# yccyenchicheng/p2pvg

Hardware: NVIDIA H100
Metric: frames/sec (train step, device-timed) MovingMNIST 64x64 seq30 (higher is better)
Workload: dtype bf16

## Files before the change

p2pvg_b200/csrc/conv_gemm.cu:

```cuda

#include "tc_common.cuh"

namespace {

using namespace tc;

struct Geom {
  int N, H, W;
  int Ck, Cn;
  int M;
  int Ntot;
  int bh128, bn128;
  int bh64, bn64;
  int bw64;
  int imgs_per_group;
  int add_bf16;
  int bres;
  int swap;
  int ks, st, sgn;
};

__device__ __forceinline__ void pix_block(int pb, int P, int H, int W, int bh, int bn, int& n0, int& y0) {
  const int HW = H * W;
  if (HW >= P) {
    const int bpi = HW / P;
    n0 = pb / bpi;
    y0 = (pb - n0 * bpi) * bh;
  } else {
    n0 = pb * bn;
    y0 = 0;
  }
}

__device__ __forceinline__ void addend_load64(float4 (&a4)[16], const float* base, long long elem_off, bool is_bf16) {
  if (is_bf16) {
    const uint4* p = reinterpret_cast<const uint4*>(reinterpret_cast<const bf16*>(base) + elem_off);
#pragma unroll
    for (int j = 0; j < 8; j++) {
      const uint4 r = p[j];
      a4[j] = make_float4(__uint_as_float(r.x), __uint_as_float(r.y), __uint_as_float(r.z), __uint_as_float(r.w));
    }
  } else {
    const float4* p = reinterpret_cast<const float4*>(base + elem_off);
#pragma unroll
    for (int j = 0; j < 16; j++) a4[j] = p[j];
  }
}
__device__ __forceinline__ void addend_add32(float (&f)[32], const float4 (&a4)[16], int h, bool is_bf16) {
  if (is_bf16) {
#pragma unroll
    for (int j = 0; j < 4; j++) {
      const float4 r = a4[4 * h + j];
      float v[8];
      unpack16<bf16>(make_uint4(__float_as_uint(r.x), __float_as_uint(r.y), __float_as_uint(r.z), __float_as_uint(r.w)), v);
#pragma unroll
      for (int i = 0; i < 8; i++) f[8 * j + i] += v[i];
    }
  } else {
#pragma unroll
    for (int j = 0; j < 8; j++) {
      const float4 x4 = a4[8 * h + j];
      f[4 * j] += x4.x; f[4 * j + 1] += x4.y; f[4 * j + 2] += x4.z; f[4 * j + 3] += x4.w;
    }
  }
}

template <int KIND, int BN, bool STAT, bool EVAL = false>
__global__ void __launch_bounds__(NUM_THREADS, 1)
conv_gemm_kernel(const __grid_constant__ CUtensorMap tmA, const __grid_constant__ CUtensorMap tmB, void* __restrict__ Cv, int c_bf16,
                 long long ldc, Geom g, int accumulate, const float* __restrict__ bias, const float* __restrict__ addend,
                 const int* __restrict__ grp_src, float* __restrict__ partial, int kb_per_split, int splits,
                 float2* __restrict__ stat_partial, const float* __restrict__ eval_scale, const float* __restrict__ eval_shift, int act) {
  using C_ = Cfg<BN>;
  constexpr bool A_MN = (KIND == 1), B_MN = (KIND != 0);
  extern __shared__ uint8_t smem_raw[];
  const Smem sm = smem_setup<BN>(smem_raw);
  const bool bres = (KIND == 0) && (BN == 64) && g.bres != 0;

  const int warp = threadIdx.x >> 5, lane = threadIdx.x & 31;
  const int tiles_m = (g.M + BLOCK_M - 1) / BLOCK_M, tiles_n = (g.Ntot + BN - 1) / BN;
  const int tiles_mn = tiles_m * tiles_n;
  const int phases = (KIND == 2) ? 4 : 1;
  const int num_tiles = tiles_mn * splits * phases;
  const int cchunks = g.Ck / 64;
  const int nkb_total = (KIND == 0) ? g.ks * g.ks * cchunks : (KIND == 2) ? 4 * cchunks : (g.N * g.H * g.W + 63) / 64;

  if (warp >= 8) {
    regs_producer();
    if (warp == 8 && lane == 0) {
      uint32_t it = 0;
      if (bres) {
        mbar_expect_tx(sm.bres_bar, (uint32_t)(g.ks * g.ks) * 64 * 128);
        for (int tap = 0; tap < g.ks * g.ks; tap++) tma_load_2d(&tmB, sm.bres_bar, sm.ring + tap * 64 * 128, tap * 64, 0);
      }
      for (int t = blockIdx.x; t < num_tiles; t += gridDim.x) {
        const int ph = (KIND == 2) ? (t & 3) : 0;
        const int t2 = (KIND == 2) ? (t >> 2) : t;
        const int z = (splits == 1) ? 0 : t2 / tiles_mn, r = t2 - z * tiles_mn;
        const int mt = (tiles_n == 1) ? r : r / tiles_n, nt = (tiles_n == 1) ? 0 : r - mt * tiles_n;
        const int n0 = nt * BN;
        const int kb0 = z * kb_per_split, kb1 = min(kb0 + kb_per_split, nkb_total);
        int pn0 = 0, py0 = 0;
        if (KIND != 1) pix_block(mt, 128, g.H, g.W, g.bh128, g.bn128, pn0, py0);
        const int pa = ph >> 1, pb_ = ph & 1;
        int kn0 = 0, ky0 = 0, kx0 = 0;
        int t_kh = 0, t_kw = 0, t_cc = 0;
        int qc0[BN / 64], qdx[BN / 64], qdy[BN / 64];
        int mc0[2] = {0, 0}, mdx[2] = {0, 0}, mdy[2] = {0, 0};
        if (KIND == 1) {
          if (g.bw64 < g.W) {
            const int per_row = g.W / g.bw64;
            const int rowi = kb0 / per_row;
            kx0 = (kb0 - rowi * per_row) * g.bw64;
            kn0 = rowi / g.H;
            ky0 = rowi - kn0 * g.H;
          } else {
            pix_block(kb0, 64, g.H, g.W, g.bh64, g.bn64, kn0, ky0);
          }
#pragma unroll
          for (int q = 0; q < BN / 64; q++) {
            const int nb = n0 + 64 * q;
            const int tap = nb / g.Cn;
            const int kh = tap / g.ks;
            qc0[q] = nb - tap * g.Cn;
            qdx[q] = tap - kh * g.ks - 1;
            qdy[q] = kh - 1;
          }
          if (g.swap) {
#pragma unroll
            for (int q = 0; q < 2; q++) {
              const int mb = mt * BLOCK_M + 64 * q;
              int tap = mb / g.Cn;
              if (tap >= g.ks * g.ks) tap = g.ks * g.ks - 1;
              const int kh = tap / g.ks;
              mc0[q] = mb < g.M ? mb - tap * g.Cn : 0;
              mdx[q] = tap - kh * g.ks - 1;
              mdy[q] = kh - 1;
            }
          }
        }
        for (int kb = kb0; kb < kb1; kb++, it++) {
          const int s = bres ? (int)(it % BRES_STAGES) : (int)(it % C_::STAGES);
          const uint32_t par = (bres ? (it / BRES_STAGES) : (it / C_::STAGES)) & 1;
          mbar_wait(&sm.empty_bar[s], par ^ 1);
          uint8_t* sa = bres ? sm.ring + BRES_B_BYTES + s * A_STAGE_BYTES : sm.ring + s * C_::STAGE_BYTES;
          uint8_t* sb = sa + A_STAGE_BYTES;
          mbar_expect_tx(&sm.full_bar[s], bres ? A_STAGE_BYTES : C_::STAGE_BYTES);
          if (KIND == 0) {
            tma_load_4d(&tmA, &sm.full_bar[s], sa, t_cc * 64, g.sgn * (t_kw - 1), g.st * py0 + g.sgn * (t_kh - 1), pn0);
            if (!bres) tma_load_2d(&tmB, &sm.full_bar[s], sb, kb * 64, n0);
            if (++t_cc == cchunks) { t_cc = 0; if (++t_kw == g.ks) { t_kw = 0; t_kh++; } }
          } else if (KIND == 2) {
            const int tq = t_kh, c0 = t_cc * 64;
            if (++t_cc == cchunks) { t_cc = 0; t_kh++; }
            const int i = tq >> 1, j = tq & 1;
            const int dy = i == 0 ? 0 : (pa ? 1 : -1), ky = i == 0 ? pa + 1 : (pa ? 0 : 3);
            const int dx = j == 0 ? 0 : (pb_ ? 1 : -1), kx = j == 0 ? pb_ + 1 : (pb_ ? 0 : 3);
            tma_load_4d(&tmA, &sm.full_bar[s], sa, c0, dx, py0 + dy, pn0);
#pragma unroll
            for (int q = 0; q < BN / 64; q++)
              tma_load_2d(&tmB, &sm.full_bar[s], sb + q * 64 * 128, (ky * 4 + kx) * g.Cn + n0 + 64 * q, c0);
          } else {
            const int m0 = mt * BLOCK_M;
            if (g.swap) {
              tma_load_4d(&tmA, &sm.full_bar[s], sa, mc0[0], g.st * kx0 + mdx[0], g.st * ky0 + mdy[0], kn0);
              tma_load_4d(&tmA, &sm.full_bar[s], sa + 64 * 128, mc0[1], g.st * kx0 + mdx[1], g.st * ky0 + mdy[1], kn0);
#pragma unroll
              for (int q = 0; q < BN / 64; q++) tma_load_2d(&tmB, &sm.full_bar[s], sb + q * 64 * 128, n0 + 64 * q, kb * 64);
            } else {
              tma_load_2d(&tmA, &sm.full_bar[s], sa, m0, kb * 64);
              tma_load_2d(&tmA, &sm.full_bar[s], sa + 64 * 128, m0 + 64, kb * 64);
#pragma unroll
              for (int q = 0; q < BN / 64; q++)
                tma_load_4d(&tmB, &sm.full_bar[s], sb + q * 64 * 128, qc0[q], g.st * kx0 + qdx[q], g.st * ky0 + qdy[q], kn0);
            }
            if (g.bw64 < g.W) {
              kx0 += g.bw64;
              if (kx0 >= g.W) { kx0 = 0; if (++ky0 >= g.H) { ky0 = 0; kn0++; } }
            } else if (g.H * g.W >= 64) {
              ky0 += g.bh64;
              if (ky0 >= g.H) { ky0 = 0; kn0++; }
            } else {
              kn0 += g.bn64;
            }
          }
        }
      }
    }
  } else if (warp >= 4) {
    regs_worker();
    mma_loop<false, BN, A_MN, B_MN>(sm, num_tiles, tiles_mn, splits, kb_per_split, nkb_total, bres);
  } else {
    regs_worker();
    const int q = warp;
    __shared__ float bias_s[2 * BN];
    __shared__ float2 stat_s[STAT ? 2 * 4 * BN : 1];
    constexpr bool do_stat = STAT;
    __shared__ float ev_s[EVAL ? 2 * 2 * BN : 1];
    const bool row_major_store = !STAT && !EVAL && KIND != 1 && c_bf16 && !accumulate && addend == nullptr;
    uint32_t lt = 0;
    for (int t = blockIdx.x; t < num_tiles; t += gridDim.x, lt++) {
      const int ph = (KIND == 2) ? (t & 3) : 0;
      const int t2 = (KIND == 2) ? (t >> 2) : t;
      const int z = (splits == 1) ? 0 : t2 / tiles_mn, r = t2 - z * tiles_mn;
      const int mt = (tiles_n == 1) ? r : r / tiles_n, nt = (tiles_n == 1) ? 0 : r - mt * tiles_n;
      const int n0 = nt * BN;
      const uint32_t acc = lt & 1;
      const int rt = q * 32 + lane;
      long long out_row = (long long)mt * BLOCK_M + rt;
      long long add_row = 0;
      bool row_ok = out_row < g.M;
      if (KIND == 2) {
        int pn0, py0;
        pix_block(mt, 128, g.H, g.W, g.bh128, g.bn128, pn0, py0);
        const int HW = g.H * g.W;
        int nn, yy, xx;
        if (HW >= 128) { nn = 0; yy = rt / g.W; xx = rt - yy * g.W; }
        else { nn = rt / HW; const int rem = rt - nn * HW; yy = rem / g.W; xx = rem - yy * g.W; }
        const int n = pn0 + nn, y = py0 + yy;
        row_ok = (n < g.N) && (y < g.H);
        const int oy = 2 * y + (ph >> 1), ox = 2 * xx + (ph & 1);
        out_row = ((long long)n * (2 * g.H) + oy) * (2 * g.W) + ox;
        if (addend && row_ok) {
          const int n2 = grp_src[n / g.imgs_per_group] * g.imgs_per_group + (n % g.imgs_per_group);
          add_row = ((long long)n2 * (2 * g.H) + oy) * (2 * g.W) + ox;
        }
      }
      if (KIND == 0 && addend && row_ok) {
        const int HW = g.H * g.W;
        const int n = (int)(out_row / HW);
        const int n2 = grp_src[n / g.imgs_per_group] * g.imgs_per_group + (n % g.imgs_per_group);
        add_row = (long long)n2 * HW + (out_row - (long long)n * HW);
      }
      if (EVAL) {
        stage_cols<BN>(ev_s + acc * 2 * BN, eval_scale, n0, g.Ntot);
        stage_cols<BN>(ev_s + acc * 2 * BN + BN, eval_shift, n0, g.Ntot);
        if (bias == nullptr) epi_bar_sync();
      }
      if (bias != nullptr) {
        stage_cols<BN>(bias_s + acc * BN, bias, n0, g.Ntot);
        epi_bar_sync();
      }
      const bool use_add = (KIND != 1) && addend != nullptr && row_ok;
      const long long aoff0 = add_row * g.Ntot + n0;
      const bool abf = g.add_bf16 != 0;
      if (row_major_store) {
        constexpr int LPR = BN / 8, RPI = 32 / LPR;
        const int sub = lane / LPR, cl = (lane % LPR) * 8;
        const bool col_ok = n0 + cl < g.Ntot;
        bf16* cbase = reinterpret_cast<bf16*>(Cv) + n0 + cl;
        mbar_wait(sm.acc_full_bar, lt & 1);
#pragma unroll
        for (int i = 0; i < 32 / RPI; i++) {
          const int src = i * RPI + sub;
          const long long orow = __shfl_sync(0xffffffffu, out_row, src);
          const bool ok = __shfl_sync(0xffffffffu, (int)row_ok, src) != 0;
          const float* s = sm.accs + (q * 32 + src) * C_::ACC_LD + cl;
          const float4 x0 = *reinterpret_cast<const float4*>(s), x1 = *reinterpret_cast<const float4*>(s + 4);
          if (i == 32 / RPI - 1) {
            __syncwarp();
            if (lane == 0) mbar_arrive(sm.acc_empty_bar);
          }
          if (!ok || !col_ok) continue;
          float f[8] = {x0.x, x0.y, x0.z, x0.w, x1.x, x1.y, x1.z, x1.w};
          if (bias) {
#pragma unroll
            for (int j = 0; j < 8; j++) f[j] += bias_s[acc * BN + cl + j];
          }
          *reinterpret_cast<uint4*>(cbase + orow * ldc) = pack16<bf16>(f);
        }
        continue;
      }
      float4 a4[16];
      if (use_add) addend_load64(a4, addend, aoff0, abf);
      mbar_wait(sm.acc_full_bar, lt & 1);
#pragma unroll 1
      for (int pr = 0; pr < BN / 64; pr++) {
        if (pr > 0 && use_add) addend_load64(a4, addend, aoff0 + pr * 64, abf);
#pragma unroll
        for (int h = 0; h < 2; h++) {
          const int c = pr * 2 + h;
          float f[32];
          read_chunk<BN>(sm, rt, c, f);
          const int nbase = n0 + c * 32;
          if (nbase >= g.Ntot) continue;
          if (!row_ok && !do_stat) continue;
          if (KIND == 1 && partial != nullptr) {
            float* dst = partial + ((long long)z * g.M + out_row) * g.Ntot + nbase;
#pragma unroll
            for (int j = 0; j < 32; j += 8)
              st_global_256(dst + j, __float_as_uint(f[j]), __float_as_uint(f[j + 1]), __float_as_uint(f[j + 2]), __float_as_uint(f[j + 3]),
                            __float_as_uint(f[j + 4]), __float_as_uint(f[j + 5]), __float_as_uint(f[j + 6]), __float_as_uint(f[j + 7]));
            continue;
          }
          if (bias) add_staged32(f, bias_s + acc * BN + c * 32);
          if (use_add) addend_add32(f, a4, h, abf);
          if (EVAL) {
            const float* sc = ev_s + acc * 2 * BN + c * 32;
#pragma unroll
            for (int j = 0; j < 32; j++) {
              float y = fmaf(f[j], sc[j], sc[BN + j]);
              if (act == P2PVG_ACT_LRELU) y = y > 0.f ? y : 0.2f * y;
              else if (act == P2PVG_ACT_TANH) y = tanhf(y);
              f[j] = y;
            }
          }
          if (STAT) {
            float s1[32], s2[32];
#pragma unroll
            for (int j = 0; j < 32; j++) {
              const float r = row_ok ? (c_bf16 ? bf16_round(f[j]) : f[j]) : 0.f;
              s1[j] = r;
              s2[j] = r * r;
            }
            const float cs = warp_colsum32(s1, lane), cq = warp_colsum32(s2, lane);
            stat_s[(acc * 4 + q) * BN + c * 32 + lane] = make_float2(cs, cq);
            if (!row_ok) continue;
          }
          if (c_bf16) store_row32<bf16, false>(reinterpret_cast<bf16*>(Cv) + out_row * ldc + nbase, f, accumulate, 32);
          else store_row32<float, false>(reinterpret_cast<float*>(Cv) + out_row * ldc + nbase, f, accumulate, 32);
        }
      }
      if (STAT) {
        epi_bar_sync();
        float2* dst = stat_partial + ((long long)mt * phases + ph) * g.Ntot + n0;
        for (int i = q * 32 + lane; i < BN; i += 128) {
          if (n0 + i >= g.Ntot) continue;
          const float2 a = stat_s[(acc * 4 + 0) * BN + i], b = stat_s[(acc * 4 + 1) * BN + i];
          const float2 c2 = stat_s[(acc * 4 + 2) * BN + i], d = stat_s[(acc * 4 + 3) * BN + i];
          dst[i] = make_float2((a.x + b.x) + (c2.x + d.x), (a.y + b.y) + (c2.y + d.y));
        }
      }
    }
  }
}

int map4d(CUtensorMap* m, const void* base, int N, int Hm, int Wm, int C, int bw, int bh, int bn, int s) {
  cuuint64_t dims[4] = {(cuuint64_t)C, (cuuint64_t)Wm, (cuuint64_t)Hm, (cuuint64_t)N};
  cuuint64_t strides[3] = {(cuuint64_t)C * 2, (cuuint64_t)Wm * C * 2, (cuuint64_t)Hm * Wm * C * 2};
  cuuint32_t box[4] = {64, (cuuint32_t)(bw * s), (cuuint32_t)(bh * s), (cuuint32_t)bn};
  cuuint32_t es[4] = {1, (cuuint32_t)s, (cuuint32_t)s, 1};
  CUresult r = driver().encode(m, CU_TENSOR_MAP_DATA_TYPE_BFLOAT16, 4, const_cast<void*>(base), dims, strides, box, es, CU_TENSOR_MAP_INTERLEAVE_NONE,
                     CU_TENSOR_MAP_SWIZZLE_128B, CU_TENSOR_MAP_L2_PROMOTION_L2_256B, CU_TENSOR_MAP_FLOAT_OOB_FILL_NONE);
  if (r != CUDA_SUCCESS) {
    p2pvg_set_error("conv_gemm: 4-D tensor map failed (%d): N=%d H=%d W=%d C=%d box=(%d,%d,%d) s=%d", (int)r, N, Hm, Wm, C, bw, bh, bn, s);
    return P2PVG_ERR_CUDA;
  }
  return P2PVG_OK;
}

bool box_for(int P, int H, int W, int& bh, int& bn) {
  const int HW = H * W;
  if (HW >= P) {
    if (P % W != 0 || (H % (P / W)) != 0) return false;
    bh = P / W;
    bn = 1;
  } else {
    if (P % HW != 0) return false;
    bh = H;
    bn = P / HW;
  }
  return bh * 2 <= 256 && W * 2 <= 256 && bn <= 256;
}

struct EvalEpi {
  const float* scale = nullptr;
  const float* shift = nullptr;
  int act = 0;
};

template <int KIND, int BN, bool STAT, bool EVAL>
int launch_t(const CUtensorMap& ta, const CUtensorMap& tb, void* C, int c_dtype, long long ldc, const Geom& g, int accumulate,
             const float* bias, const float* addend, const int* grp_src, float* partial, int splits, int kb_per_split, cudaStream_t st,
             float2* stat_partial, const EvalEpi& ev) {
  const long long tiles = (long long)cdiv(g.M, BLOCK_M) * cdiv(g.Ntot, BN) * splits * (KIND == 2 ? 4 : 1);
  return launch_persistent<conv_gemm_kernel<KIND, BN, STAT, EVAL>, BN>(tiles, st, "conv_gemm", ta, tb, C, (int)(c_dtype == P2PVG_BF16), ldc, g,
                                                                       accumulate, bias, addend, grp_src, partial, kb_per_split, splits,
                                                                       stat_partial, ev.scale, ev.shift, ev.act);
}

template <int KIND, int BN>
int launch(const CUtensorMap& ta, const CUtensorMap& tb, void* C, int c_dtype, long long ldc, const Geom& g, int accumulate,
           const float* bias, const float* addend, const int* grp_src, float* partial, int splits, int kb_per_split, cudaStream_t st,
           float2* stat_partial = nullptr, const EvalEpi& ev = EvalEpi()) {
  if (KIND != 1 && ev.scale != nullptr) return launch_t<KIND, BN, false, (KIND != 1)>(ta, tb, C, c_dtype, ldc, g, accumulate, bias, addend, grp_src, partial, splits, kb_per_split, st, nullptr, ev);
  if (KIND != 1 && stat_partial != nullptr) return launch_t<KIND, BN, (KIND != 1), false>(ta, tb, C, c_dtype, ldc, g, accumulate, bias, addend, grp_src, partial, splits, kb_per_split, st, stat_partial, ev);
  return launch_t<KIND, BN, false, false>(ta, tb, C, c_dtype, ldc, g, accumulate, bias, addend, grp_src, partial, splits, kb_per_split, st, nullptr, ev);
}

}

int p2pvg_conv_gemm_impl(int kind, const void* a, const void* b, long long ldb, void* c, int c_dtype, long long ldc, int N, int H, int W,
                         int Ck, int Cn, int Cm, const float* bias, const float* addend, const int* grp_src, int imgs_per_group,
                         int accumulate, void* ws, size_t ws_bytes, void* stat_partial_v, int addend_dtype, const float* eval_scale,
                         const float* eval_shift, int act, cudaStream_t st) {
  float2* stat_partial = reinterpret_cast<float2*>(stat_partial_v);
  EvalEpi ev;
  ev.scale = eval_scale; ev.shift = eval_shift; ev.act = act;
  P2PVG_REQUIRE(driver().encode != nullptr, P2PVG_ERR_UNSUPPORTED, "conv_gemm: cuTensorMapEncodeTiled unavailable");
  P2PVG_REQUIRE(kind >= 0 && kind <= 5, P2PVG_ERR_BAD_ARG, "conv_gemm: bad kind %d", kind);
  if (eval_scale != nullptr) {
    P2PVG_REQUIRE(kind == 0 || kind == 2, P2PVG_ERR_BAD_ARG, "conv_gemm: the eval-BatchNorm epilogue belongs to kinds 0 and 2");
    P2PVG_REQUIRE(eval_shift != nullptr, P2PVG_ERR_BAD_ARG, "conv_gemm: eval_scale without eval_shift");
    P2PVG_REQUIRE(stat_partial == nullptr, P2PVG_ERR_BAD_ARG, "conv_gemm: the eval-BatchNorm epilogue excludes fwd_stat_partial");
    P2PVG_REQUIRE(!accumulate, P2PVG_ERR_BAD_ARG, "conv_gemm: the eval-BatchNorm epilogue does not accumulate");
    P2PVG_REQUIRE(act == P2PVG_ACT_LRELU || act == P2PVG_ACT_TANH, P2PVG_ERR_BAD_ARG, "conv_gemm: eval epilogue act %d", act);
  }
  if (N <= 0) return P2PVG_OK;
  Geom g;
  g.N = N; g.H = H; g.W = W; g.Ck = Ck; g.Cn = Cn; g.imgs_per_group = imgs_per_group > 0 ? imgs_per_group : 1;
  g.add_bf16 = (addend != nullptr && addend_dtype == P2PVG_BF16) ? 1 : 0;
  g.swap = 0;
  g.bres = 0;
  g.ks = kind >= 3 ? 3 : 4; g.st = kind >= 3 ? 1 : 2; g.sgn = kind == 5 ? -1 : 1;
  const int taps = g.ks * g.ks;
  if (kind == 3 || kind == 5) kind = 0;
  if (kind == 4) kind = 1;
  g.bh128 = g.bn128 = g.bh64 = g.bn64 = 1;
  g.bw64 = W;
  bool ok;
  if (kind == 1) {
    if (W > 64 && W % 64 == 0 && W * g.st <= 256) { g.bw64 = 64; ok = true; }
    else ok = box_for(64, H, W, g.bh64, g.bn64);
  } else {
    ok = box_for(128, H, W, g.bh128, g.bn128);
  }
  ok = ok && (((uintptr_t)a | (uintptr_t)b | (uintptr_t)c) & 15) == 0;
  if (kind == 1) ok = ok && (Cn % 64 == 0) && (Cm % 8 == 0);
  else ok = ok && (Ck % 64 == 0) && (Cn % 32 == 0) && (ldb % 8 == 0);
  if (kind == 2 || addend != nullptr) ok = ok && (Cn % 64 == 0);
  if (!ok) {
    p2pvg_set_error("conv_gemm: shape not supported by the pixel-box tiling (kind=%d N=%d H=%d W=%d Ck=%d Cn=%d)", kind, N, H, W, Ck, Cn);
    return P2PVG_ERR_UNSUPPORTED;
  }
  CUtensorMap ta, tb;
  int rc;
  const long long pix = (long long)N * H * W;
  if (kind == 0) {
    g.M = (int)pix; g.Ntot = Cn;
    rc = map4d(&ta, a, N, g.st * H, g.st * W, Ck, W, g.bh128, g.bn128, g.st);
    if (rc) return rc;
    const int BN = Cn > 64 ? 128 : 64;
    rc = map2d(&tb, b, (long long)taps * Ck, Cn, ldb, BN);
    if (rc) return rc;
    const int nkb = taps * (Ck / 64);
    g.bres = (BN == 64 && Cn == 64 && Ck == 64 && taps <= 9) ? 1 : 0;
    if (BN == 128) return launch<0, 128>(ta, tb, c, c_dtype, ldc, g, accumulate, bias, addend, grp_src, nullptr, 1, nkb, st, stat_partial, ev);
    return launch<0, 64>(ta, tb, c, c_dtype, ldc, g, accumulate, bias, addend, grp_src, nullptr, 1, nkb, st, stat_partial, ev);
  }
  if (kind == 2) {
    g.M = (int)pix; g.Ntot = Cn;
    rc = map4d(&ta, a, N, H, W, Ck, W, g.bh128, g.bn128, 1);
    if (rc) return rc;
    rc = map2d(&tb, b, 16LL * Cn, Ck, ldb, 64);
    if (rc) return rc;
    const int nkb = 4 * (Ck / 64);
    const int BN = Cn > 64 ? 128 : 64;
    if (BN == 128) return launch<2, 128>(ta, tb, c, c_dtype, ldc, g, accumulate, bias, addend, grp_src, nullptr, 1, nkb, st, stat_partial, ev);
    return launch<2, 64>(ta, tb, c, c_dtype, ldc, g, accumulate, bias, addend, grp_src, nullptr, 1, nkb, st, stat_partial, ev);
  }
  P2PVG_REQUIRE(c_dtype == P2PVG_F32, P2PVG_ERR_BAD_ARG, "conv_gemm kind 1 writes fp32");
  P2PVG_REQUIRE(stat_partial == nullptr, P2PVG_ERR_BAD_ARG, "conv_gemm: BatchNorm statistics belong to the forward / data-gradient kinds");
  g.Ck = 64;
  const int nkb = (int)((pix + 63) / 64);
  g.swap = (Cm == 64 && nkb >= 16 && ws != nullptr && (size_t)2 * taps * Cn * Cm * sizeof(float) <= ws_bytes) ? 1 : 0;
  if (g.swap) {
    g.M = taps * Cn; g.Ntot = Cm;
    rc = map4d(&ta, b, N, g.st * H, g.st * W, Cn, g.bw64, g.bh64, g.bn64, g.st);
    if (rc) return rc;
    rc = map2d(&tb, a, Cm, pix, Cm, 64);
    if (rc) return rc;
  } else {
    g.M = Cm; g.Ntot = taps * Cn;
    rc = map2d(&ta, a, Cm, pix, Cm, 64);
    if (rc) return rc;
    rc = map4d(&tb, b, N, g.st * H, g.st * W, Cn, g.bw64, g.bh64, g.bn64, g.st);
    if (rc) return rc;
  }
  const int BN = (g.Ntot % 128 == 0) ? 128 : 64;
  const long long tiles = (long long)cdiv(g.M, BLOCK_M) * cdiv(g.Ntot, BN);
  int splits = g.swap ? 2 : 1;
  {
    double best = 1e300;
    const int maxs = nkb / 8 < 64 ? nkb / 8 : 64;
    const int smin = g.swap ? 2 : 1;
    for (int s = smin; s <= (maxs < smin ? smin : maxs); s++) {
      const int kb = cdiv(nkb, s), se = cdiv(nkb, kb);
      if (se > 1 && (ws == nullptr || (size_t)se * g.M * g.Ntot * sizeof(float) > ws_bytes)) continue;
      const long long rounds = cdiv((long long)tiles * se, driver().sms);
      double cost = (double)rounds * (kb + 8.0);
      if (se > 1) cost += (double)se * g.M * g.Ntot * 8.0 / 6.0e12 / (0.22e-6 * BN / 128);
      if (cost < best) { best = cost; splits = se; }
    }
  }
  int kbps = cdiv(nkb, splits);
  splits = cdiv(nkb, kbps);
  float* partial = splits > 1 ? reinterpret_cast<float*>(ws) : nullptr;
  if (BN == 128) rc = launch<1, 128>(ta, tb, c, c_dtype, ldc, g, accumulate, nullptr, nullptr, nullptr, partial, splits, kbps, st);
  else rc = launch<1, 64>(ta, tb, c, c_dtype, ldc, g, accumulate, nullptr, nullptr, nullptr, partial, splits, kbps, st);
  if (rc) return rc;
  if (splits > 1)
    return p2pvg_splitk_reduce(partial, splits, c, P2PVG_F32, ldc, Cm, taps * Cn, accumulate, nullptr, nullptr, 0, g.swap, st);
  P2PVG_REQUIRE(!g.swap, P2PVG_ERR_UNSUPPORTED, "conv_gemm kind 1 (swapped roles) needs the split-K workspace");
  return P2PVG_OK;
}
```

p2pvg_b200/csrc/tc_common.cuh:

```cuda
#pragma once
#include <cuda.h>

#include "common.cuh"

namespace tc {

__device__ __forceinline__ uint32_t smem_u32(const void* p) { return (uint32_t)__cvta_generic_to_shared(p); }

__device__ __forceinline__ void mbar_init(uint64_t* bar, uint32_t count) {
  asm volatile("mbarrier.init.shared::cta.b64 [%0], %1;" ::"r"(smem_u32(bar)), "r"(count));
}
__device__ __forceinline__ void mbar_expect_tx(uint64_t* bar, uint32_t bytes) {
  asm volatile("mbarrier.arrive.expect_tx.shared::cta.b64 _, [%0], %1;" ::"r"(smem_u32(bar)), "r"(bytes) : "memory");
}
__device__ __forceinline__ void mbar_wait(uint64_t* bar, uint32_t parity) {
  asm volatile(
      "{\n\t"
      ".reg .pred P1;\n\t"
      "WAIT_LOOP:\n\t"
      "mbarrier.try_wait.parity.shared::cta.b64 P1, [%0], %1;\n\t"
      "@P1 bra DONE;\n\t"
      "bra WAIT_LOOP;\n\t"
      "DONE:\n\t"
      "}" ::"r"(smem_u32(bar)),
      "r"(parity)
      : "memory");
}
__device__ __forceinline__ void tma_load_2d(const CUtensorMap* desc, uint64_t* bar, void* smem_dst, int c0, int c1) {
  asm volatile(
      "cp.async.bulk.tensor.2d.shared::cluster.global.mbarrier::complete_tx::bytes [%0], [%1, {%3, %4}], [%2];" ::"r"(
          smem_u32(smem_dst)),
      "l"(reinterpret_cast<uint64_t>(desc)), "r"(smem_u32(bar)), "r"(c0), "r"(c1)
      : "memory");
}
__device__ __forceinline__ void wgmma_fence() { asm volatile("wgmma.fence.sync.aligned;" ::: "memory"); }
__device__ __forceinline__ void wgmma_commit() { asm volatile("wgmma.commit_group.sync.aligned;" ::: "memory"); }
template <int N>
__device__ __forceinline__ void wgmma_wait() { asm volatile("wgmma.wait_group.sync.aligned %0;" ::"n"(N) : "memory"); }
template <int N>
__device__ __forceinline__ void fence_regs(float (&r)[N]) {
#pragma unroll
  for (int i = 0; i < N; i++) asm volatile("" : "+f"(r[i])::"memory");
}
template <int TA, int TB>
__device__ __forceinline__ void wgmma_bf16_n64(float* d, uint64_t desc_a, uint64_t desc_b, uint32_t scale_d) {
  asm volatile(
      "{\n\t.reg .pred p;\n\tsetp.ne.b32 p, %34, 0;\n\t"
      "wgmma.mma_async.sync.aligned.m64n64k16.f32.bf16.bf16 "
      "{%0, %1, %2, %3, %4, %5, %6, %7, %8, %9, %10, %11, %12, %13, %14, %15, %16, %17, %18, %19, %20, %21, %22, %23, %24, %25, %26, %27, %28, %29, %30, %31}, %32, %33, p, 1, 1, %35, %36;\n\t}"
      : "+f"(d[0]), "+f"(d[1]), "+f"(d[2]), "+f"(d[3]), "+f"(d[4]), "+f"(d[5]), "+f"(d[6]), "+f"(d[7]), "+f"(d[8]), "+f"(d[9]), "+f"(d[10]), "+f"(d[11]), "+f"(d[12]), "+f"(d[13]), "+f"(d[14]), "+f"(d[15]), "+f"(d[16]), "+f"(d[17]), "+f"(d[18]), "+f"(d[19]), "+f"(d[20]), "+f"(d[21]), "+f"(d[22]), "+f"(d[23]), "+f"(d[24]), "+f"(d[25]), "+f"(d[26]), "+f"(d[27]), "+f"(d[28]), "+f"(d[29]), "+f"(d[30]), "+f"(d[31])
      : "l"(desc_a), "l"(desc_b), "r"(scale_d), "n"(TA), "n"(TB));
}
template <int TA, int TB>
__device__ __forceinline__ void wgmma_bf16_n128(float* d, uint64_t desc_a, uint64_t desc_b, uint32_t scale_d) {
  asm volatile(
      "{\n\t.reg .pred p;\n\tsetp.ne.b32 p, %66, 0;\n\t"
      "wgmma.mma_async.sync.aligned.m64n128k16.f32.bf16.bf16 "
      "{%0, %1, %2, %3, %4, %5, %6, %7, %8, %9, %10, %11, %12, %13, %14, %15, %16, %17, %18, %19, %20, %21, %22, %23, %24, %25, %26, %27, %28, %29, %30, %31, %32, %33, %34, %35, %36, %37, %38, %39, %40, %41, %42, %43, %44, %45, %46, %47, %48, %49, %50, %51, %52, %53, %54, %55, %56, %57, %58, %59, %60, %61, %62, %63}, %64, %65, p, 1, 1, %67, %68;\n\t}"
      : "+f"(d[0]), "+f"(d[1]), "+f"(d[2]), "+f"(d[3]), "+f"(d[4]), "+f"(d[5]), "+f"(d[6]), "+f"(d[7]), "+f"(d[8]), "+f"(d[9]), "+f"(d[10]), "+f"(d[11]), "+f"(d[12]), "+f"(d[13]), "+f"(d[14]), "+f"(d[15]), "+f"(d[16]), "+f"(d[17]), "+f"(d[18]), "+f"(d[19]), "+f"(d[20]), "+f"(d[21]), "+f"(d[22]), "+f"(d[23]), "+f"(d[24]), "+f"(d[25]), "+f"(d[26]), "+f"(d[27]), "+f"(d[28]), "+f"(d[29]), "+f"(d[30]), "+f"(d[31]), "+f"(d[32]), "+f"(d[33]), "+f"(d[34]), "+f"(d[35]), "+f"(d[36]), "+f"(d[37]), "+f"(d[38]), "+f"(d[39]), "+f"(d[40]), "+f"(d[41]), "+f"(d[42]), "+f"(d[43]), "+f"(d[44]), "+f"(d[45]), "+f"(d[46]), "+f"(d[47]), "+f"(d[48]), "+f"(d[49]), "+f"(d[50]), "+f"(d[51]), "+f"(d[52]), "+f"(d[53]), "+f"(d[54]), "+f"(d[55]), "+f"(d[56]), "+f"(d[57]), "+f"(d[58]), "+f"(d[59]), "+f"(d[60]), "+f"(d[61]), "+f"(d[62]), "+f"(d[63])
      : "l"(desc_a), "l"(desc_b), "r"(scale_d), "n"(TA), "n"(TB));
}
__device__ __forceinline__ void wgmma_tf32_n64(float* d, uint64_t desc_a, uint64_t desc_b, uint32_t scale_d) {
  asm volatile(
      "{\n\t.reg .pred p;\n\tsetp.ne.b32 p, %34, 0;\n\t"
      "wgmma.mma_async.sync.aligned.m64n64k8.f32.tf32.tf32 "
      "{%0, %1, %2, %3, %4, %5, %6, %7, %8, %9, %10, %11, %12, %13, %14, %15, %16, %17, %18, %19, %20, %21, %22, %23, %24, %25, %26, %27, %28, %29, %30, %31}, %32, %33, p, 1, 1;\n\t}"
      : "+f"(d[0]), "+f"(d[1]), "+f"(d[2]), "+f"(d[3]), "+f"(d[4]), "+f"(d[5]), "+f"(d[6]), "+f"(d[7]), "+f"(d[8]), "+f"(d[9]), "+f"(d[10]), "+f"(d[11]), "+f"(d[12]), "+f"(d[13]), "+f"(d[14]), "+f"(d[15]), "+f"(d[16]), "+f"(d[17]), "+f"(d[18]), "+f"(d[19]), "+f"(d[20]), "+f"(d[21]), "+f"(d[22]), "+f"(d[23]), "+f"(d[24]), "+f"(d[25]), "+f"(d[26]), "+f"(d[27]), "+f"(d[28]), "+f"(d[29]), "+f"(d[30]), "+f"(d[31])
      : "l"(desc_a), "l"(desc_b), "r"(scale_d));
}
__device__ __forceinline__ void wgmma_tf32_n128(float* d, uint64_t desc_a, uint64_t desc_b, uint32_t scale_d) {
  asm volatile(
      "{\n\t.reg .pred p;\n\tsetp.ne.b32 p, %66, 0;\n\t"
      "wgmma.mma_async.sync.aligned.m64n128k8.f32.tf32.tf32 "
      "{%0, %1, %2, %3, %4, %5, %6, %7, %8, %9, %10, %11, %12, %13, %14, %15, %16, %17, %18, %19, %20, %21, %22, %23, %24, %25, %26, %27, %28, %29, %30, %31, %32, %33, %34, %35, %36, %37, %38, %39, %40, %41, %42, %43, %44, %45, %46, %47, %48, %49, %50, %51, %52, %53, %54, %55, %56, %57, %58, %59, %60, %61, %62, %63}, %64, %65, p, 1, 1;\n\t}"
      : "+f"(d[0]), "+f"(d[1]), "+f"(d[2]), "+f"(d[3]), "+f"(d[4]), "+f"(d[5]), "+f"(d[6]), "+f"(d[7]), "+f"(d[8]), "+f"(d[9]), "+f"(d[10]), "+f"(d[11]), "+f"(d[12]), "+f"(d[13]), "+f"(d[14]), "+f"(d[15]), "+f"(d[16]), "+f"(d[17]), "+f"(d[18]), "+f"(d[19]), "+f"(d[20]), "+f"(d[21]), "+f"(d[22]), "+f"(d[23]), "+f"(d[24]), "+f"(d[25]), "+f"(d[26]), "+f"(d[27]), "+f"(d[28]), "+f"(d[29]), "+f"(d[30]), "+f"(d[31]), "+f"(d[32]), "+f"(d[33]), "+f"(d[34]), "+f"(d[35]), "+f"(d[36]), "+f"(d[37]), "+f"(d[38]), "+f"(d[39]), "+f"(d[40]), "+f"(d[41]), "+f"(d[42]), "+f"(d[43]), "+f"(d[44]), "+f"(d[45]), "+f"(d[46]), "+f"(d[47]), "+f"(d[48]), "+f"(d[49]), "+f"(d[50]), "+f"(d[51]), "+f"(d[52]), "+f"(d[53]), "+f"(d[54]), "+f"(d[55]), "+f"(d[56]), "+f"(d[57]), "+f"(d[58]), "+f"(d[59]), "+f"(d[60]), "+f"(d[61]), "+f"(d[62]), "+f"(d[63])
      : "l"(desc_a), "l"(desc_b), "r"(scale_d));
}
__device__ __forceinline__ void st_global_256(void* p, uint32_t a, uint32_t b, uint32_t c, uint32_t d, uint32_t e, uint32_t f, uint32_t g,
                                              uint32_t h) {
  uint4* q = reinterpret_cast<uint4*>(p);
  q[0] = make_uint4(a, b, c, d);
  q[1] = make_uint4(e, f, g, h);
}
__device__ __forceinline__ uint32_t pack_bf16x2(float lo, float hi) {
  __nv_bfloat162 v = __floats2bfloat162_rn(lo, hi);
  return *reinterpret_cast<uint32_t*>(&v);
}
__device__ __forceinline__ void regs_producer() { asm volatile("setmaxnreg.dec.sync.aligned.u32 40;"); }
__device__ __forceinline__ void regs_worker() { asm volatile("setmaxnreg.inc.sync.aligned.u32 232;"); }
__device__ __forceinline__ void epi_bar_sync() { asm volatile("bar.sync 1, 128;" ::: "memory"); }

__device__ __forceinline__ uint64_t make_desc(uint32_t smem_addr, uint32_t lbo_bytes, uint32_t sbo_bytes) {
  uint64_t d = 0;
  d |= (uint64_t)((smem_addr >> 4) & 0x3FFF);
  d |= (uint64_t)((lbo_bytes >> 4) & 0x3FFF) << 16;
  d |= (uint64_t)((sbo_bytes >> 4) & 0x3FFF) << 32;
  d |= (uint64_t)1 << 62;
  return d;
}

template <bool TF32, int BN, bool A_MN, bool B_MN>
__device__ __forceinline__ void wgmma_kblock(float (&acc)[2][BN / 2], uint64_t da, uint64_t db, bool first) {
  constexpr int UMMA_K = TF32 ? 8 : 16;
  constexpr int KSTEPS = 4;
  constexpr uint32_t A_STEP = (A_MN ? UMMA_K * 128 : 32) >> 4, B_STEP = (B_MN ? UMMA_K * 128 : 32) >> 4;
#pragma unroll
  for (int k = 0; k < KSTEPS; k++) {
    const uint32_t sc = (first && k == 0) ? 0u : 1u;
#pragma unroll
    for (int h = 0; h < 2; h++) {
      const uint64_t a = da + (uint64_t)(h * (8192 >> 4) + k * A_STEP), b = db + (uint64_t)(k * B_STEP);
      if constexpr (TF32) {
        if constexpr (BN == 128) wgmma_tf32_n128(acc[h], a, b, sc);
        else wgmma_tf32_n64(acc[h], a, b, sc);
      } else {
        if constexpr (BN == 128) wgmma_bf16_n128<A_MN ? 1 : 0, B_MN ? 1 : 0>(acc[h], a, b, sc);
        else wgmma_bf16_n64<A_MN ? 1 : 0, B_MN ? 1 : 0>(acc[h], a, b, sc);
      }
    }
  }
}

template <int BN>
__device__ __forceinline__ void acc_to_smem(const float (&acc)[2][BN / 2], float* buf, int ld, int t) {
  const int w = t >> 5, l = t & 31;
#pragma unroll
  for (int h = 0; h < 2; h++) {
    float* r0 = buf + (64 * h + 16 * w + (l >> 2)) * ld + 2 * (l & 3);
#pragma unroll
    for (int j = 0; j < BN / 8; j++) {
      *reinterpret_cast<float2*>(r0 + 8 * j) = make_float2(acc[h][4 * j], acc[h][4 * j + 1]);
      *reinterpret_cast<float2*>(r0 + 8 * ld + 8 * j) = make_float2(acc[h][4 * j + 2], acc[h][4 * j + 3]);
    }
  }
}

__device__ __forceinline__ void mbar_arrive(uint64_t* bar) {
  asm volatile("mbarrier.arrive.shared::cta.b64 _, [%0];" ::"r"(smem_u32(bar)) : "memory");
}
__device__ __forceinline__ void tma_load_4d(const CUtensorMap* desc, uint64_t* bar, void* smem_dst, int c0, int c1, int c2, int c3) {
  asm volatile(
      "cp.async.bulk.tensor.4d.shared::cluster.global.mbarrier::complete_tx::bytes [%0], [%1, {%3, %4, %5, %6}], [%2];" ::"r"(
          smem_u32(smem_dst)),
      "l"(reinterpret_cast<uint64_t>(desc)), "r"(smem_u32(bar)), "r"(c0), "r"(c1), "r"(c2), "r"(c3)
      : "memory");
}

template <int OFF>
__device__ __forceinline__ void colsum_stage(float (&v)[32], int lane) {
  const bool upper = (lane & OFF) != 0;
#pragma unroll
  for (int j = 0; j < OFF; j++) {
    const float send = upper ? v[j] : v[j + OFF];
    const float keep = upper ? v[j + OFF] : v[j];
    v[j] = keep + __shfl_xor_sync(0xffffffffu, send, OFF);
  }
  if constexpr (OFF > 1) colsum_stage<OFF / 2>(v, lane);
}
__device__ __forceinline__ float warp_colsum32(float (&v)[32], int lane) {
  colsum_stage<16>(v, lane);
  return v[0];
}
__device__ __forceinline__ float bf16_round(float x) { return __bfloat162float(__float2bfloat16_rn(x)); }

constexpr int BLOCK_M = 128;
constexpr int ROW_BYTES = 128;
constexpr int A_STAGE_BYTES = BLOCK_M * ROW_BYTES;
constexpr int NUM_THREADS = 384;

template <int BN> struct Cfg {
  static constexpr int B_STAGE_BYTES = BN * ROW_BYTES;
  static constexpr int STAGE_BYTES = A_STAGE_BYTES + B_STAGE_BYTES;
  static constexpr int STAGES = (BN == 128) ? 4 : 7;
  static constexpr int ACC_LD = BN + 4;
  static constexpr int ACC_BYTES = BLOCK_M * ACC_LD * 4;
  static constexpr int SMEM_BYTES = STAGES * STAGE_BYTES + ACC_BYTES + 1024  + 512 ;
};

constexpr int BRES_B_BYTES = 9 * 64 * 128, BRES_STAGES = 6;
static_assert(BRES_B_BYTES + BRES_STAGES * A_STAGE_BYTES <= Cfg<64>::STAGES * Cfg<64>::STAGE_BYTES, "resident weights + A ring");

struct Smem {
  uint8_t* ring;
  float* accs;
  uint64_t *full_bar, *empty_bar, *acc_full_bar, *acc_empty_bar;
  uint64_t* bres_bar;
};

template <int BN>
__device__ __forceinline__ Smem smem_setup(uint8_t* smem_raw) {
  using C_ = Cfg<BN>;
  Smem s;
  s.ring = reinterpret_cast<uint8_t*>((reinterpret_cast<uintptr_t>(smem_raw) + 1023) & ~(uintptr_t)1023);
  s.accs = reinterpret_cast<float*>(s.ring + C_::STAGES * C_::STAGE_BYTES);
  s.full_bar = reinterpret_cast<uint64_t*>(s.ring + C_::STAGES * C_::STAGE_BYTES + C_::ACC_BYTES);
  s.empty_bar = s.full_bar + C_::STAGES;
  s.acc_full_bar = s.empty_bar + C_::STAGES;
  s.acc_empty_bar = s.acc_full_bar + 1;
  s.bres_bar = s.acc_empty_bar + 1;
  if (threadIdx.x == 0) {
    for (int i = 0; i < C_::STAGES; i++) {
      mbar_init(&s.full_bar[i], 1);
      mbar_init(&s.empty_bar[i], 128);
    }
    mbar_init(s.acc_full_bar, 128);
    mbar_init(s.acc_empty_bar, 4);
    mbar_init(s.bres_bar, 1);
    asm volatile("fence.mbarrier_init.release.cluster;" ::: "memory");
  }
  __syncthreads();
  return s;
}

template <bool TF32, int BN, bool A_MN, bool B_MN>
__device__ __forceinline__ void mma_loop(const Smem& sm, int num_tiles, int tiles_mn, int splits, int kb_per_split, int nkb_total,
                                         bool bres) {
  using C_ = Cfg<BN>;
  const int wt = threadIdx.x - 128;
  const uint32_t smem0 = smem_u32(sm.ring);
  const uint64_t da0 = A_MN ? make_desc(smem0, 64 * 128, 1024) : make_desc(smem0, 0, 1024);
  const uint64_t db0 = B_MN ? make_desc(smem0 + A_STAGE_BYTES, 64 * 128, 1024) : make_desc(smem0 + A_STAGE_BYTES, 0, 1024);
  uint32_t it = 0, lt = 0;
  if (bres) mbar_wait(sm.bres_bar, 0);
  const uint64_t da0r = make_desc(smem0 + BRES_B_BYTES, 0, 1024), db0r = make_desc(smem0, 0, 1024);
  float acc[2][BN / 2];
  for (int t = blockIdx.x; t < num_tiles; t += gridDim.x, lt++) {
    const int z = (splits == 1) ? 0 : t / tiles_mn;
    const int kb0 = z * kb_per_split, kb1 = min(kb0 + kb_per_split, nkb_total);
    int prev = -1;
    for (int kb = kb0; kb < kb1; kb++, it++) {
      const int s = bres ? (int)(it % BRES_STAGES) : (int)(it % C_::STAGES);
      const uint32_t par = (bres ? (it / BRES_STAGES) : (it / C_::STAGES)) & 1;
      mbar_wait(&sm.full_bar[s], par);
      const uint64_t stage_off = (uint64_t)((uint32_t)s * (uint32_t)(C_::STAGE_BYTES >> 4));
      const uint64_t a_off = bres ? (uint64_t)((uint32_t)s * (uint32_t)(A_STAGE_BYTES >> 4)) : stage_off;
      const uint64_t b_off = bres ? (uint64_t)((uint32_t)kb * (uint32_t)((64 * 128) >> 4)) : stage_off;
      fence_regs(acc[0]);
      fence_regs(acc[1]);
      wgmma_fence();
      wgmma_kblock<TF32, BN, A_MN, B_MN>(acc, (bres ? da0r : da0) + a_off, (bres ? db0r : db0) + b_off, kb == kb0);
      wgmma_commit();
      wgmma_wait<1>();
      fence_regs(acc[0]);
      fence_regs(acc[1]);
      if (prev >= 0) mbar_arrive(&sm.empty_bar[prev]);
      prev = s;
    }
    wgmma_wait<0>();
    fence_regs(acc[0]);
    fence_regs(acc[1]);
    if (prev >= 0) mbar_arrive(&sm.empty_bar[prev]);
    mbar_wait(sm.acc_empty_bar, (lt & 1) ^ 1);
    acc_to_smem<BN>(acc, sm.accs, C_::ACC_LD, wt);
    mbar_arrive(sm.acc_full_bar);
  }
}

template <int BN>
__device__ __forceinline__ void stage_cols(float* dst, const float* src, int n0, int N) {
  for (int i = threadIdx.x; i < BN; i += 128) dst[i] = (n0 + i < N) ? src[n0 + i] : 0.f;
}

template <int BN>
__device__ __forceinline__ void read_chunk(const Smem& sm, int row, int c, float (&f)[32]) {
  const float* src = sm.accs + row * Cfg<BN>::ACC_LD + c * 32;
#pragma unroll
  for (int j = 0; j < 32; j += 4) {
    const float4 x = *reinterpret_cast<const float4*>(src + j);
    f[j] = x.x; f[j + 1] = x.y; f[j + 2] = x.z; f[j + 3] = x.w;
  }
  if (c == BN / 32 - 1) {
    __syncwarp();
    if ((threadIdx.x & 31) == 0) mbar_arrive(sm.acc_empty_bar);
  }
}

__device__ __forceinline__ void add_staged32(float (&f)[32], const float* s) {
#pragma unroll
  for (int j = 0; j < 32; j += 4) {
    const float4 b4 = *reinterpret_cast<const float4*>(s + j);
    f[j] += b4.x; f[j + 1] += b4.y; f[j + 2] += b4.z; f[j + 3] += b4.w;
  }
}

template <typename T, bool TAIL>
__device__ __forceinline__ void add_row32(float (&f)[32], const T* row, int ncols) {
#pragma unroll
  for (int j = 0; j < 32; j++)
    if (!TAIL || j < ncols) f[j] += ld_f<T>(row + j);
}

template <typename T, bool TAIL>
__device__ __forceinline__ void store_row32(T* crow, float (&f)[32], int accumulate, int ncols) {
  if (accumulate) add_row32<T, TAIL>(f, crow, ncols);
  const bool vec = !TAIL || (ncols >= 32 && (reinterpret_cast<uintptr_t>(crow) & 15) == 0);
  if (vec && (reinterpret_cast<uintptr_t>(crow) & 31) == 0) {
    if constexpr (sizeof(T) == 2) {
#pragma unroll
      for (int j = 0; j < 32; j += 16)
        st_global_256(crow + j, pack_bf16x2(f[j], f[j + 1]), pack_bf16x2(f[j + 2], f[j + 3]), pack_bf16x2(f[j + 4], f[j + 5]),
                      pack_bf16x2(f[j + 6], f[j + 7]), pack_bf16x2(f[j + 8], f[j + 9]), pack_bf16x2(f[j + 10], f[j + 11]),
                      pack_bf16x2(f[j + 12], f[j + 13]), pack_bf16x2(f[j + 14], f[j + 15]));
    } else {
#pragma unroll
      for (int j = 0; j < 32; j += 8)
        st_global_256(crow + j, __float_as_uint(f[j]), __float_as_uint(f[j + 1]), __float_as_uint(f[j + 2]), __float_as_uint(f[j + 3]),
                      __float_as_uint(f[j + 4]), __float_as_uint(f[j + 5]), __float_as_uint(f[j + 6]), __float_as_uint(f[j + 7]));
    }
  } else if (vec) {
    if constexpr (sizeof(T) == 2) {
#pragma unroll
      for (int j = 0; j < 32; j += 8)
        *reinterpret_cast<uint4*>(crow + j) =
            make_uint4(pack_bf16x2(f[j], f[j + 1]), pack_bf16x2(f[j + 2], f[j + 3]), pack_bf16x2(f[j + 4], f[j + 5]), pack_bf16x2(f[j + 6], f[j + 7]));
    } else {
#pragma unroll
      for (int j = 0; j < 32; j += 4) *reinterpret_cast<float4*>(crow + j) = make_float4(f[j], f[j + 1], f[j + 2], f[j + 3]);
    }
  } else {
#pragma unroll
    for (int j = 0; j < 32; j++)
      if (j < ncols) st_f<T>(crow + j, f[j]);
  }
}

typedef CUresult (*EncodeTiledFn)(CUtensorMap*, CUtensorMapDataType, cuuint32_t, void*, const cuuint64_t*, const cuuint64_t*,
                                  const cuuint32_t*, const cuuint32_t*, CUtensorMapInterleave, CUtensorMapSwizzle,
                                  CUtensorMapL2promotion, CUtensorMapFloatOOBfill);
struct Driver {
  EncodeTiledFn encode = nullptr;
  int sms = 132;
};

inline const Driver& driver() {
  static const Driver d = [] {
    Driver r;
    int dev = 0, sms = 0;
    if (cudaGetDevice(&dev) == cudaSuccess && cudaDeviceGetAttribute(&sms, cudaDevAttrMultiProcessorCount, dev) == cudaSuccess && sms > 0)
      r.sms = sms;
    void* fn = nullptr;
    cudaDriverEntryPointQueryResult q;
    if (cudaGetDriverEntryPoint("cuTensorMapEncodeTiled", &fn, cudaEnableDefault, &q) == cudaSuccess && q == cudaDriverEntryPointSuccess)
      r.encode = reinterpret_cast<EncodeTiledFn>(fn);
    (void)cudaGetLastError();
    return r;
  }();
  return d;
}

inline int map2d(CUtensorMap* map, const void* base, long long dim0, long long dim1, long long ld, int box1, int elem = 2) {
  cuuint64_t dims[2] = {(cuuint64_t)dim0, (cuuint64_t)dim1};
  cuuint64_t strides[1] = {(cuuint64_t)ld * elem};
  cuuint32_t box[2] = {(cuuint32_t)(ROW_BYTES / elem), (cuuint32_t)box1};
  cuuint32_t estr[2] = {1, 1};
  CUresult r = driver().encode(map, elem == 2 ? CU_TENSOR_MAP_DATA_TYPE_BFLOAT16 : CU_TENSOR_MAP_DATA_TYPE_FLOAT32, 2, const_cast<void*>(base),
                               dims, strides, box, estr, CU_TENSOR_MAP_INTERLEAVE_NONE, CU_TENSOR_MAP_SWIZZLE_128B,
                               CU_TENSOR_MAP_L2_PROMOTION_L2_256B, CU_TENSOR_MAP_FLOAT_OOB_FILL_NONE);
  if (r != CUDA_SUCCESS) {
    p2pvg_set_error("cuTensorMapEncodeTiled failed (%d): base=%p dims=(%lld,%lld) ld=%lld box1=%d", (int)r, base, dim0, dim1, ld, box1);
    return P2PVG_ERR_CUDA;
  }
  return P2PVG_OK;
}

template <auto KERN, int BN, typename... Args>
int launch_persistent(long long tiles, cudaStream_t st, const char* what, Args... args) {
  static bool smem_attr_set = false;
  if (!smem_attr_set) {
    const cudaError_t e = cudaFuncSetAttribute(KERN, cudaFuncAttributeMaxDynamicSharedMemorySize, Cfg<BN>::SMEM_BYTES);
    if (e != cudaSuccess) {
      p2pvg_set_error("%s: cudaFuncSetAttribute: %s", what, cudaGetErrorString(e));
      return P2PVG_ERR_CUDA;
    }
    smem_attr_set = true;
  }
  const int sms = driver().sms;
  KERN<<<(int)(tiles < sms ? tiles : sms), NUM_THREADS, Cfg<BN>::SMEM_BYTES, st>>>(args...);
  return p2pvg_check_launch(what);
}

}
```

Baseline: 211,500.

## Add 256-row tile path for transposed-conv GEMM with swapped wgmma operands

```diff
diff --git a/p2pvg_b200/csrc/conv_gemm.cu b/p2pvg_b200/csrc/conv_gemm.cu
--- a/p2pvg_b200/csrc/conv_gemm.cu
+++ b/p2pvg_b200/csrc/conv_gemm.cu
@@ -10,7 +10,7 @@
   int Ck, Cn;
   int M;
   int Ntot;
-  int bh128, bn128;
+  int bhm, bnm;
   int bh64, bn64;
   int bw64;
   int imgs_per_group;
@@ -65,20 +65,21 @@
   }
 }
 
-template <int KIND, int BN, bool STAT, bool EVAL = false>
+template <int KIND, int BM, int BN, bool STAT, bool EVAL>
 __global__ void __launch_bounds__(NUM_THREADS, 1)
 conv_gemm_kernel(const __grid_constant__ CUtensorMap tmA, const __grid_constant__ CUtensorMap tmB, void* __restrict__ Cv, int c_bf16,
                  long long ldc, Geom g, int accumulate, const float* __restrict__ bias, const float* __restrict__ addend,
                  const int* __restrict__ grp_src, float* __restrict__ partial, int kb_per_split, int splits,
                  float2* __restrict__ stat_partial, const float* __restrict__ eval_scale, const float* __restrict__ eval_shift, int act) {
-  using C_ = Cfg<BN>;
+  static_assert(BM == 128 || (KIND == 2 && !STAT && !EVAL), "256-row tiles: kind 2 without statistics or eval epilogue");
+  using C_ = Cfg<BN, BM>;
   constexpr bool A_MN = (KIND == 1), B_MN = (KIND != 0);
   extern __shared__ uint8_t smem_raw[];
-  const Smem sm = smem_setup<BN>(smem_raw);
+  const Smem sm = smem_setup<BN, BM>(smem_raw);
   const bool bres = (KIND == 0) && (BN == 64) && g.bres != 0;
 
   const int warp = threadIdx.x >> 5, lane = threadIdx.x & 31;
-  const int tiles_m = (g.M + BLOCK_M - 1) / BLOCK_M, tiles_n = (g.Ntot + BN - 1) / BN;
+  const int tiles_m = (g.M + BM - 1) / BM, tiles_n = (g.Ntot + BN - 1) / BN;
   const int tiles_mn = tiles_m * tiles_n;
   const int phases = (KIND == 2) ? 4 : 1;
   const int num_tiles = tiles_mn * splits * phases;
@@ -101,7 +102,7 @@
         const int n0 = nt * BN;
         const int kb0 = z * kb_per_split, kb1 = min(kb0 + kb_per_split, nkb_total);
         int pn0 = 0, py0 = 0;
-        if (KIND != 1) pix_block(mt, 128, g.H, g.W, g.bh128, g.bn128, pn0, py0);
+        if (KIND != 1) pix_block(mt, BM, g.H, g.W, g.bhm, g.bnm, pn0, py0);
         const int pa = ph >> 1, pb_ = ph & 1;
         int kn0 = 0, ky0 = 0, kx0 = 0;
         int t_kh = 0, t_kw = 0, t_cc = 0;
@@ -129,7 +130,7 @@
           if (g.swap) {
 #pragma unroll
             for (int q = 0; q < 2; q++) {
-              const int mb = mt * BLOCK_M + 64 * q;
+              const int mb = mt * BM + 64 * q;
               int tap = mb / g.Cn;
               if (tap >= g.ks * g.ks) tap = g.ks * g.ks - 1;
               const int kh = tap / g.ks;
@@ -144,7 +145,7 @@
           const uint32_t par = (bres ? (it / BRES_STAGES) : (it / C_::STAGES)) & 1;
           mbar_wait(&sm.empty_bar[s], par ^ 1);
           uint8_t* sa = bres ? sm.ring + BRES_B_BYTES + s * A_STAGE_BYTES : sm.ring + s * C_::STAGE_BYTES;
-          uint8_t* sb = sa + A_STAGE_BYTES;
+          uint8_t* sb = sa + C_::A_STAGE_BYTES;
           mbar_expect_tx(&sm.full_bar[s], bres ? A_STAGE_BYTES : C_::STAGE_BYTES);
           if (KIND == 0) {
             tma_load_4d(&tmA, &sm.full_bar[s], sa, t_cc * 64, g.sgn * (t_kw - 1), g.st * py0 + g.sgn * (t_kh - 1), pn0);
@@ -161,7 +162,7 @@
             for (int q = 0; q < BN / 64; q++)
               tma_load_2d(&tmB, &sm.full_bar[s], sb + q * 64 * 128, (ky * 4 + kx) * g.Cn + n0 + 64 * q, c0);
           } else {
-            const int m0 = mt * BLOCK_M;
+            const int m0 = mt * BM;
             if (g.swap) {
               tma_load_4d(&tmA, &sm.full_bar[s], sa, mc0[0], g.st * kx0 + mdx[0], g.st * ky0 + mdy[0], kn0);
               tma_load_4d(&tmA, &sm.full_bar[s], sa + 64 * 128, mc0[1], g.st * kx0 + mdx[1], g.st * ky0 + mdy[1], kn0);
@@ -189,7 +190,7 @@
     }
   } else if (warp >= 4) {
     regs_worker();
-    mma_loop<false, BN, A_MN, B_MN>(sm, num_tiles, tiles_mn, splits, kb_per_split, nkb_total, bres);
+    mma_loop<false, BN, A_MN, B_MN, BM>(sm, num_tiles, tiles_mn, splits, kb_per_split, nkb_total, bres);
   } else {
     regs_worker();
     const int q = warp;
@@ -197,8 +198,8 @@
     __shared__ float2 stat_s[STAT ? 2 * 4 * BN : 1];
     constexpr bool do_stat = STAT;
     __shared__ float ev_s[EVAL ? 2 * 2 * BN : 1];
-    const bool row_major_store = !STAT && !EVAL && KIND != 1 && c_bf16 && !accumulate && addend == nullptr;
-    uint32_t lt = 0;
+    const bool row_major_store = !STAT && !EVAL && KIND != 1 && c_bf16 && !accumulate && (addend == nullptr || g.add_bf16);
+    uint32_t lt = 0, lh = 0;
     for (int t = blockIdx.x; t < num_tiles; t += gridDim.x, lt++) {
       const int ph = (KIND == 2) ? (t & 3) : 0;
       const int t2 = (KIND == 2) ? (t >> 2) : t;
@@ -206,32 +207,33 @@
       const int mt = (tiles_n == 1) ? r : r / tiles_n, nt = (tiles_n == 1) ? 0 : r - mt * tiles_n;
       const int n0 = nt * BN;
       const uint32_t acc = lt & 1;
-      const int rt = q * 32 + lane;
-      long long out_row = (long long)mt * BLOCK_M + rt;
-      long long add_row = 0;
-      bool row_ok = out_row < g.M;
-      if (KIND == 2) {
-        int pn0, py0;
-        pix_block(mt, 128, g.H, g.W, g.bh128, g.bn128, pn0, py0);
-        const int HW = g.H * g.W;
-        int nn, yy, xx;
-        if (HW >= 128) { nn = 0; yy = rt / g.W; xx = rt - yy * g.W; }
-        else { nn = rt / HW; const int rem = rt - nn * HW; yy = rem / g.W; xx = rem - yy * g.W; }
-        const int n = pn0 + nn, y = py0 + yy;
-        row_ok = (n < g.N) && (y < g.H);
-        const int oy = 2 * y + (ph >> 1), ox = 2 * xx + (ph & 1);
-        out_row = ((long long)n * (2 * g.H) + oy) * (2 * g.W) + ox;
-        if (addend && row_ok) {
+      int pn0 = 0, py0 = 0;
+      if (KIND == 2) pix_block(mt, BM, g.H, g.W, g.bhm, g.bnm, pn0, py0);
+      auto row_of = [&](int rt, long long& out_row, long long& add_row, bool& row_ok) {
+        out_row = (long long)mt * BM + rt;
+        add_row = 0;
+        row_ok = out_row < g.M;
+        if (KIND == 2) {
+          const int HW = g.H * g.W;
+          int nn, yy, xx;
+          if (HW >= BM) { nn = 0; yy = rt / g.W; xx = rt - yy * g.W; }
+          else { nn = rt / HW; const int rem = rt - nn * HW; yy = rem / g.W; xx = rem - yy * g.W; }
+          const int n = pn0 + nn, y = py0 + yy;
+          row_ok = (n < g.N) && (y < g.H);
+          const int oy = 2 * y + (ph >> 1), ox = 2 * xx + (ph & 1);
+          out_row = ((long long)n * (2 * g.H) + oy) * (2 * g.W) + ox;
+          if (addend && row_ok) {
+            const int n2 = grp_src[n / g.imgs_per_group] * g.imgs_per_group + (n % g.imgs_per_group);
+            add_row = ((long long)n2 * (2 * g.H) + oy) * (2 * g.W) + ox;
+          }
+        }
+        if (KIND == 0 && addend && row_ok) {
+          const int HW = g.H * g.W;
+          const int n = (int)(out_row / HW);
           const int n2 = grp_src[n / g.imgs_per_group] * g.imgs_per_group + (n % g.imgs_per_group);
-          add_row = ((long long)n2 * (2 * g.H) + oy) * (2 * g.W) + ox;
-        }
-      }
-      if (KIND == 0 && addend && row_ok) {
-        const int HW = g.H * g.W;
-        const int n = (int)(out_row / HW);
-        const int n2 = grp_src[n / g.imgs_per_group] * g.imgs_per_group + (n % g.imgs_per_group);
-        add_row = (long long)n2 * HW + (out_row - (long long)n * HW);
-      }
+          add_row = (long long)n2 * HW + (out_row - (long long)n * HW);
+        }
+      };
       if (EVAL) {
         stage_cols<BN>(ev_s + acc * 2 * BN, eval_scale, n0, g.Ntot);
         stage_cols<BN>(ev_s + acc * 2 * BN + BN, eval_shift, n0, g.Ntot);
@@ -241,84 +243,128 @@
         stage_cols<BN>(bias_s + acc * BN, bias, n0, g.Ntot);
         epi_bar_sync();
       }
-      const bool use_add = (KIND != 1) && addend != nullptr && row_ok;
-      const long long aoff0 = add_row * g.Ntot + n0;
       const bool abf = g.add_bf16 != 0;
       if (row_major_store) {
-        constexpr int LPR = BN / 8, RPI = 32 / LPR;
+        constexpr int LPR = BN / 8, RPI = 32 / LPR, STEPS = 32 / RPI, HALVES = BM / 128;
         const int sub = lane / LPR, cl = (lane % LPR) * 8;
         const bool col_ok = n0 + cl < g.Ntot;
         bf16* cbase = reinterpret_cast<bf16*>(Cv) + n0 + cl;
-        mbar_wait(sm.acc_full_bar, lt & 1);
-#pragma unroll
-        for (int i = 0; i < 32 / RPI; i++) {
-          const int src = i * RPI + sub;
-          const long long orow = __shfl_sync(0xffffffffu, out_row, src);
-          const bool ok = __shfl_sync(0xffffffffu, (int)row_ok, src) != 0;
-          const float* s = sm.accs + (q * 32 + src) * C_::ACC_LD + cl;
-          const float4 x0 = *reinterpret_cast<const float4*>(s), x1 = *reinterpret_cast<const float4*>(s + 4);
-          if (i == 32 / RPI - 1) {
-            __syncwarp();
-            if (lane == 0) mbar_arrive(sm.acc_empty_bar);
-          }
-          if (!ok || !col_ok) continue;
-          float f[8] = {x0.x, x0.y, x0.z, x0.w, x1.x, x1.y, x1.z, x1.w};
-          if (bias) {
-#pragma unroll
-            for (int j = 0; j < 8; j++) f[j] += bias_s[acc * BN + cl + j];
-          }
-          *reinterpret_cast<uint4*>(cbase + orow * ldc) = pack16<bf16>(f);
+        long long orow_h[HALVES];
+        bool ok_h[HALVES];
+        uint4 av[HALVES * STEPS];
+#pragma unroll
+        for (int hf = 0; hf < HALVES; hf++) {
+          long long arow_h;
+          row_of(hf * 128 + q * 32 + lane, orow_h[hf], arow_h, ok_h[hf]);
+          if (addend != nullptr) {
+            const bf16* abase = reinterpret_cast<const bf16*>(addend) + n0 + cl;
+#pragma unroll
+            for (int i = 0; i < STEPS; i++) {
+              const int src = i * RPI + sub;
+              const long long arow = __shfl_sync(0xffffffffu, arow_h, src);
+              const bool aok = __shfl_sync(0xffffffffu, (int)ok_h[hf], src) != 0;
+              av[hf * STEPS + i] = (aok && col_ok) ? *reinterpret_cast<const uint4*>(abase + arow * g.Ntot) : make_uint4(0, 0, 0, 0);
+            }
+          }
+        }
+        constexpr int CH = STEPS < 8 ? STEPS : 8;
+#pragma unroll
+        for (int hf = 0; hf < HALVES; hf++, lh++) {
+          mbar_wait(sm.acc_full_bar, lh & 1);
+#pragma unroll
+          for (int c0 = 0; c0 < STEPS; c0 += CH) {
+            float4 x[CH][2];
+#pragma unroll
+            for (int k = 0; k < CH; k++) {
+              const float* s = sm.accs + (q * 32 + (c0 + k) * RPI + sub) * C_::ACC_LD + cl;
+              x[k][0] = *reinterpret_cast<const float4*>(s);
+              x[k][1] = *reinterpret_cast<const float4*>(s + 4);
+            }
+            if (c0 + CH == STEPS) {
+              __syncwarp();
+              if (lane == 0) mbar_arrive(sm.acc_empty_bar);
+            }
+#pragma unroll
+            for (int k = 0; k < CH; k++) {
+              const int i = c0 + k, src = i * RPI + sub;
+              const long long orow = __shfl_sync(0xffffffffu, orow_h[hf], src);
+              const bool ok = __shfl_sync(0xffffffffu, (int)ok_h[hf], src) != 0;
+              if (!ok || !col_ok) continue;
+              const float4 x0 = x[k][0], x1 = x[k][1];
+              float f[8] = {x0.x, x0.y, x0.z, x0.w, x1.x, x1.y, x1.z, x1.w};
+              if (bias) {
+#pragma unroll
+                for (int j = 0; j < 8; j++) f[j] += bias_s[acc * BN + cl + j];
+              }
+              if (addend != nullptr) {
+                float a[8];
+                unpack16<bf16>(av[hf * STEPS + i], a);
+#pragma unroll
+                for (int j = 0; j < 8; j++) f[j] += a[j];
+              }
+              *reinterpret_cast<uint4*>(cbase + orow * ldc) = pack16<bf16>(f);
+            }
+          }
         }
         continue;
       }
-      float4 a4[16];
-      if (use_add) addend_load64(a4, addend, aoff0, abf);
-      mbar_wait(sm.acc_full_bar, lt & 1);
 #pragma unroll 1
-      for (int pr = 0; pr < BN / 64; pr++) {
-        if (pr > 0 && use_add) addend_load64(a4, addend, aoff0 + pr * 64, abf);
-#pragma unroll
-        for (int h = 0; h < 2; h++) {
-          const int c = pr * 2 + h;
-          float f[32];
-          read_chunk<BN>(sm, rt, c, f);
-          const int nbase = n0 + c * 32;
-          if (nbase >= g.Ntot) continue;
-          if (!row_ok && !do_stat) continue;
-          if (KIND == 1 && partial != nullptr) {
-            float* dst = partial + ((long long)z * g.M + out_row) * g.Ntot + nbase;
-#pragma unroll
-            for (int j = 0; j < 32; j += 8)
-              st_global_256(dst + j, __float_as_uint(f[j]), __float_as_uint(f[j + 1]), __float_as_uint(f[j + 2]), __float_as_uint(f[j + 3]),
-                            __float_as_uint(f[j + 4]), __float_as_uint(f[j + 5]), __float_as_uint(f[j + 6]), __float_as_uint(f[j + 7]));
-            continue;
-          }
-          if (bias) add_staged32(f, bias_s + acc * BN + c * 32);
-          if (use_add) addend_add32(f, a4, h, abf);
-          if (EVAL) {
-            const float* sc = ev_s + acc * 2 * BN + c * 32;
-#pragma unroll
-            for (int j = 0; j < 32; j++) {
-              float y = fmaf(f[j], sc[j], sc[BN + j]);
-              if (act == P2PVG_ACT_LRELU) y = y > 0.f ? y : 0.2f * y;
-              else if (act == P2PVG_ACT_TANH) y = tanhf(y);
-              f[j] = y;
-            }
-          }
-          if (STAT) {
-            float s1[32], s2[32];
-#pragma unroll
-            for (int j = 0; j < 32; j++) {
-              const float r = row_ok ? (c_bf16 ? bf16_round(f[j]) : f[j]) : 0.f;
-              s1[j] = r;
-              s2[j] = r * r;
-            }
-            const float cs = warp_colsum32(s1, lane), cq = warp_colsum32(s2, lane);
-            stat_s[(acc * 4 + q) * BN + c * 32 + lane] = make_float2(cs, cq);
-            if (!row_ok) continue;
-          }
-          if (c_bf16) store_row32<bf16, false>(reinterpret_cast<bf16*>(Cv) + out_row * ldc + nbase, f, accumulate, 32);
-          else store_row32<float, false>(reinterpret_cast<float*>(Cv) + out_row * ldc + nbase, f, accumulate, 32);
+      for (int hf = 0; hf < BM / 128; hf++, lh++) {
+        const int rs = q * 32 + lane;
+        long long out_row, add_row;
+        bool row_ok;
+        row_of(hf * 128 + rs, out_row, add_row, row_ok);
+        const bool use_add = (KIND != 1) && addend != nullptr && row_ok;
+        const long long aoff0 = add_row * g.Ntot + n0;
+        float4 a4[16];
+        if (use_add) addend_load64(a4, addend, aoff0, abf);
+        mbar_wait(sm.acc_full_bar, lh & 1);
+#pragma unroll 1
+        for (int pr = 0; pr < BN / 64; pr++) {
+          if (pr > 0 && use_add) addend_load64(a4, addend, aoff0 + pr * 64, abf);
+#pragma unroll
+          for (int h = 0; h < 2; h++) {
+            const int c = pr * 2 + h;
+            float f[32];
+            read_chunk<BN>(sm, rs, c, f);
+            const int nbase = n0 + c * 32;
+            if (nbase >= g.Ntot) continue;
+            if (!row_ok && !do_stat) continue;
+            if (KIND == 1 && partial != nullptr) {
+              float* dst = partial + ((long long)z * g.M + out_row) * g.Ntot + nbase;
+#pragma unroll
+              for (int j = 0; j < 32; j += 8)
+                st_global_256(dst + j, __float_as_uint(f[j]), __float_as_uint(f[j + 1]), __float_as_uint(f[j + 2]), __float_as_uint(f[j + 3]),
+                              __float_as_uint(f[j + 4]), __float_as_uint(f[j + 5]), __float_as_uint(f[j + 6]), __float_as_uint(f[j + 7]));
+              continue;
+            }
+            if (bias) add_staged32(f, bias_s + acc * BN + c * 32);
+            if (use_add) addend_add32(f, a4, h, abf);
+            if (EVAL) {
+              const float* sc = ev_s + acc * 2 * BN + c * 32;
+#pragma unroll
+              for (int j = 0; j < 32; j++) {
+                float y = fmaf(f[j], sc[j], sc[BN + j]);
+                if (act == P2PVG_ACT_LRELU) y = y > 0.f ? y : 0.2f * y;
+                else if (act == P2PVG_ACT_TANH) y = tanhf(y);
+                f[j] = y;
+              }
+            }
+            if (STAT) {
+              float s1[32], s2[32];
+#pragma unroll
+              for (int j = 0; j < 32; j++) {
+                const float r = row_ok ? (c_bf16 ? bf16_round(f[j]) : f[j]) : 0.f;
+                s1[j] = r;
+                s2[j] = r * r;
+              }
+              const float cs = warp_colsum32(s1, lane), cq = warp_colsum32(s2, lane);
+              stat_s[(acc * 4 + q) * BN + c * 32 + lane] = make_float2(cs, cq);
+              if (!row_ok) continue;
+            }
+            if (c_bf16) store_row32<bf16, false>(reinterpret_cast<bf16*>(Cv) + out_row * ldc + nbase, f, accumulate, 32);
+            else store_row32<float, false>(reinterpret_cast<float*>(Cv) + out_row * ldc + nbase, f, accumulate, 32);
+          }
         }
       }
       if (STAT) {
@@ -369,23 +415,25 @@
   int act = 0;
 };
 
-template <int KIND, int BN, bool STAT, bool EVAL>
+template <int KIND, int BM, int BN, bool STAT, bool EVAL>
 int launch_t(const CUtensorMap& ta, const CUtensorMap& tb, void* C, int c_dtype, long long ldc, const Geom& g, int accumulate,
              const float* bias, const float* addend, const int* grp_src, float* partial, int splits, int kb_per_split, cudaStream_t st,
              float2* stat_partial, const EvalEpi& ev) {
-  const long long tiles = (long long)cdiv(g.M, BLOCK_M) * cdiv(g.Ntot, BN) * splits * (KIND == 2 ? 4 : 1);
-  return launch_persistent<conv_gemm_kernel<KIND, BN, STAT, EVAL>, BN>(tiles, st, "conv_gemm", ta, tb, C, (int)(c_dtype == P2PVG_BF16), ldc, g,
-                                                                       accumulate, bias, addend, grp_src, partial, kb_per_split, splits,
-                                                                       stat_partial, ev.scale, ev.shift, ev.act);
-}
-
-template <int KIND, int BN>
+  const long long tiles = (long long)cdiv(g.M, BM) * cdiv(g.Ntot, BN) * splits * (KIND == 2 ? 4 : 1);
+  return launch_persistent<conv_gemm_kernel<KIND, BM, BN, STAT, EVAL>, BN, BM>(tiles, st, "conv_gemm", ta, tb, C, (int)(c_dtype == P2PVG_BF16),
+                                                                               ldc, g, accumulate, bias, addend, grp_src, partial, kb_per_split,
+                                                                               splits, stat_partial, ev.scale, ev.shift, ev.act);
+}
+
+template <int KIND, int BN, int BM = BLOCK_M>
 int launch(const CUtensorMap& ta, const CUtensorMap& tb, void* C, int c_dtype, long long ldc, const Geom& g, int accumulate,
            const float* bias, const float* addend, const int* grp_src, float* partial, int splits, int kb_per_split, cudaStream_t st,
            float2* stat_partial = nullptr, const EvalEpi& ev = EvalEpi()) {
-  if (KIND != 1 && ev.scale != nullptr) return launch_t<KIND, BN, false, (KIND != 1)>(ta, tb, C, c_dtype, ldc, g, accumulate, bias, addend, grp_src, partial, splits, kb_per_split, st, nullptr, ev);
-  if (KIND != 1 && stat_partial != nullptr) return launch_t<KIND, BN, (KIND != 1), false>(ta, tb, C, c_dtype, ldc, g, accumulate, bias, addend, grp_src, partial, splits, kb_per_split, st, stat_partial, ev);
-  return launch_t<KIND, BN, false, false>(ta, tb, C, c_dtype, ldc, g, accumulate, bias, addend, grp_src, partial, splits, kb_per_split, st, nullptr, ev);
+  if constexpr (KIND != 1 && BM == 128) {
+    if (ev.scale != nullptr) return launch_t<KIND, BM, BN, false, true>(ta, tb, C, c_dtype, ldc, g, accumulate, bias, addend, grp_src, partial, splits, kb_per_split, st, nullptr, ev);
+    if (stat_partial != nullptr) return launch_t<KIND, BM, BN, true, false>(ta, tb, C, c_dtype, ldc, g, accumulate, bias, addend, grp_src, partial, splits, kb_per_split, st, stat_partial, ev);
+  }
+  return launch_t<KIND, BM, BN, false, false>(ta, tb, C, c_dtype, ldc, g, accumulate, bias, addend, grp_src, partial, splits, kb_per_split, st, nullptr, ev);
 }
 
 }
@@ -416,14 +464,14 @@
   const int taps = g.ks * g.ks;
   if (kind == 3 || kind == 5) kind = 0;
   if (kind == 4) kind = 1;
-  g.bh128 = g.bn128 = g.bh64 = g.bn64 = 1;
+  g.bhm = g.bnm = g.bh64 = g.bn64 = 1;
   g.bw64 = W;
   bool ok;
   if (kind == 1) {
     if (W > 64 && W % 64 == 0 && W * g.st <= 256) { g.bw64 = 64; ok = true; }
     else ok = box_for(64, H, W, g.bh64, g.bn64);
   } else {
-    ok = box_for(128, H, W, g.bh128, g.bn128);
+    ok = box_for(128, H, W, g.bhm, g.bnm);
   }
   ok = ok && (((uintptr_t)a | (uintptr_t)b | (uintptr_t)c) & 15) == 0;
   if (kind == 1) ok = ok && (Cn % 64 == 0) && (Cm % 8 == 0);
@@ -438,7 +486,7 @@
   const long long pix = (long long)N * H * W;
   if (kind == 0) {
     g.M = (int)pix; g.Ntot = Cn;
-    rc = map4d(&ta, a, N, g.st * H, g.st * W, Ck, W, g.bh128, g.bn128, g.st);
+    rc = map4d(&ta, a, N, g.st * H, g.st * W, Ck, W, g.bhm, g.bnm, g.st);
     if (rc) return rc;
     const int BN = Cn > 64 ? 128 : 64;
     rc = map2d(&tb, b, (long long)taps * Ck, Cn, ldb, BN);
@@ -450,12 +498,16 @@
   }
   if (kind == 2) {
     g.M = (int)pix; g.Ntot = Cn;
-    rc = map4d(&ta, a, N, H, W, Ck, W, g.bh128, g.bn128, 1);
+    int bh256 = 1, bn256 = 1;
+    const bool tall = Cn == 64 && stat_partial == nullptr && eval_scale == nullptr && box_for(256, H, W, bh256, bn256);
+    if (tall) { g.bhm = bh256; g.bnm = bn256; }
+    rc = map4d(&ta, a, N, H, W, Ck, W, g.bhm, g.bnm, 1);
     if (rc) return rc;
     rc = map2d(&tb, b, 16LL * Cn, Ck, ldb, 64);
     if (rc) return rc;
     const int nkb = 4 * (Ck / 64);
     const int BN = Cn > 64 ? 128 : 64;
+    if (tall) return launch<2, 64, 256>(ta, tb, c, c_dtype, ldc, g, accumulate, bias, addend, grp_src, nullptr, 1, nkb, st);
     if (BN == 128) return launch<2, 128>(ta, tb, c, c_dtype, ldc, g, accumulate, bias, addend, grp_src, nullptr, 1, nkb, st, stat_partial, ev);
     return launch<2, 64>(ta, tb, c, c_dtype, ldc, g, accumulate, bias, addend, grp_src, nullptr, 1, nkb, st, stat_partial, ev);
   }
diff --git a/p2pvg_b200/csrc/tc_common.cuh b/p2pvg_b200/csrc/tc_common.cuh
--- a/p2pvg_b200/csrc/tc_common.cuh
+++ b/p2pvg_b200/csrc/tc_common.cuh
@@ -60,6 +60,15 @@
       : "+f"(d[0]), "+f"(d[1]), "+f"(d[2]), "+f"(d[3]), "+f"(d[4]), "+f"(d[5]), "+f"(d[6]), "+f"(d[7]), "+f"(d[8]), "+f"(d[9]), "+f"(d[10]), "+f"(d[11]), "+f"(d[12]), "+f"(d[13]), "+f"(d[14]), "+f"(d[15]), "+f"(d[16]), "+f"(d[17]), "+f"(d[18]), "+f"(d[19]), "+f"(d[20]), "+f"(d[21]), "+f"(d[22]), "+f"(d[23]), "+f"(d[24]), "+f"(d[25]), "+f"(d[26]), "+f"(d[27]), "+f"(d[28]), "+f"(d[29]), "+f"(d[30]), "+f"(d[31]), "+f"(d[32]), "+f"(d[33]), "+f"(d[34]), "+f"(d[35]), "+f"(d[36]), "+f"(d[37]), "+f"(d[38]), "+f"(d[39]), "+f"(d[40]), "+f"(d[41]), "+f"(d[42]), "+f"(d[43]), "+f"(d[44]), "+f"(d[45]), "+f"(d[46]), "+f"(d[47]), "+f"(d[48]), "+f"(d[49]), "+f"(d[50]), "+f"(d[51]), "+f"(d[52]), "+f"(d[53]), "+f"(d[54]), "+f"(d[55]), "+f"(d[56]), "+f"(d[57]), "+f"(d[58]), "+f"(d[59]), "+f"(d[60]), "+f"(d[61]), "+f"(d[62]), "+f"(d[63])
       : "l"(desc_a), "l"(desc_b), "r"(scale_d), "n"(TA), "n"(TB));
 }
+template <int TA, int TB>
+__device__ __forceinline__ void wgmma_bf16_n256(float* d, uint64_t desc_a, uint64_t desc_b, uint32_t scale_d) {
+  asm volatile(
+      "{\n\t.reg .pred p;\n\tsetp.ne.b32 p, %130, 0;\n\t"
+      "wgmma.mma_async.sync.aligned.m64n256k16.f32.bf16.bf16 "
+      "{%0, %1, %2, %3, %4, %5, %6, %7, %8, %9, %10, %11, %12, %13, %14, %15, %16, %17, %18, %19, %20, %21, %22, %23, %24, %25, %26, %27, %28, %29, %30, %31, %32, %33, %34, %35, %36, %37, %38, %39, %40, %41, %42, %43, %44, %45, %46, %47, %48, %49, %50, %51, %52, %53, %54, %55, %56, %57, %58, %59, %60, %61, %62, %63, %64, %65, %66, %67, %68, %69, %70, %71, %72, %73, %74, %75, %76, %77, %78, %79, %80, %81, %82, %83, %84, %85, %86, %87, %88, %89, %90, %91, %92, %93, %94, %95, %96, %97, %98, %99, %100, %101, %102, %103, %104, %105, %106, %107, %108, %109, %110, %111, %112, %113, %114, %115, %116, %117, %118, %119, %120, %121, %122, %123, %124, %125, %126, %127}, %128, %129, p, 1, 1, %131, %132;\n\t}"
+      : "+f"(d[0]), "+f"(d[1]), "+f"(d[2]), "+f"(d[3]), "+f"(d[4]), "+f"(d[5]), "+f"(d[6]), "+f"(d[7]), "+f"(d[8]), "+f"(d[9]), "+f"(d[10]), "+f"(d[11]), "+f"(d[12]), "+f"(d[13]), "+f"(d[14]), "+f"(d[15]), "+f"(d[16]), "+f"(d[17]), "+f"(d[18]), "+f"(d[19]), "+f"(d[20]), "+f"(d[21]), "+f"(d[22]), "+f"(d[23]), "+f"(d[24]), "+f"(d[25]), "+f"(d[26]), "+f"(d[27]), "+f"(d[28]), "+f"(d[29]), "+f"(d[30]), "+f"(d[31]), "+f"(d[32]), "+f"(d[33]), "+f"(d[34]), "+f"(d[35]), "+f"(d[36]), "+f"(d[37]), "+f"(d[38]), "+f"(d[39]), "+f"(d[40]), "+f"(d[41]), "+f"(d[42]), "+f"(d[43]), "+f"(d[44]), "+f"(d[45]), "+f"(d[46]), "+f"(d[47]), "+f"(d[48]), "+f"(d[49]), "+f"(d[50]), "+f"(d[51]), "+f"(d[52]), "+f"(d[53]), "+f"(d[54]), "+f"(d[55]), "+f"(d[56]), "+f"(d[57]), "+f"(d[58]), "+f"(d[59]), "+f"(d[60]), "+f"(d[61]), "+f"(d[62]), "+f"(d[63]), "+f"(d[64]), "+f"(d[65]), "+f"(d[66]), "+f"(d[67]), "+f"(d[68]), "+f"(d[69]), "+f"(d[70]), "+f"(d[71]), "+f"(d[72]), "+f"(d[73]), "+f"(d[74]), "+f"(d[75]), "+f"(d[76]), "+f"(d[77]), "+f"(d[78]), "+f"(d[79]), "+f"(d[80]), "+f"(d[81]), "+f"(d[82]), "+f"(d[83]), "+f"(d[84]), "+f"(d[85]), "+f"(d[86]), "+f"(d[87]), "+f"(d[88]), "+f"(d[89]), "+f"(d[90]), "+f"(d[91]), "+f"(d[92]), "+f"(d[93]), "+f"(d[94]), "+f"(d[95]), "+f"(d[96]), "+f"(d[97]), "+f"(d[98]), "+f"(d[99]), "+f"(d[100]), "+f"(d[101]), "+f"(d[102]), "+f"(d[103]), "+f"(d[104]), "+f"(d[105]), "+f"(d[106]), "+f"(d[107]), "+f"(d[108]), "+f"(d[109]), "+f"(d[110]), "+f"(d[111]), "+f"(d[112]), "+f"(d[113]), "+f"(d[114]), "+f"(d[115]), "+f"(d[116]), "+f"(d[117]), "+f"(d[118]), "+f"(d[119]), "+f"(d[120]), "+f"(d[121]), "+f"(d[122]), "+f"(d[123]), "+f"(d[124]), "+f"(d[125]), "+f"(d[126]), "+f"(d[127])
+      : "l"(desc_a), "l"(desc_b), "r"(scale_d), "n"(TA), "n"(TB));
+}
 __device__ __forceinline__ void wgmma_tf32_n64(float* d, uint64_t desc_a, uint64_t desc_b, uint32_t scale_d) {
   asm volatile(
       "{\n\t.reg .pred p;\n\tsetp.ne.b32 p, %34, 0;\n\t"
@@ -99,38 +108,60 @@
   return d;
 }
 
-template <bool TF32, int BN, bool A_MN, bool B_MN>
-__device__ __forceinline__ void wgmma_kblock(float (&acc)[2][BN / 2], uint64_t da, uint64_t db, bool first) {
+template <bool TF32, int BN, bool A_MN, bool B_MN, int BM>
+__device__ __forceinline__ void wgmma_kblock(float (&acc)[BM / 64][BN / 2], uint64_t da, uint64_t db, bool first) {
   constexpr int UMMA_K = TF32 ? 8 : 16;
   constexpr int KSTEPS = 4;
   constexpr uint32_t A_STEP = (A_MN ? UMMA_K * 128 : 32) >> 4, B_STEP = (B_MN ? UMMA_K * 128 : 32) >> 4;
-#pragma unroll
-  for (int k = 0; k < KSTEPS; k++) {
-    const uint32_t sc = (first && k == 0) ? 0u : 1u;
+  if constexpr (BM == 256) {
+    static_assert(!TF32 && BN == 64 && !A_MN && B_MN, "256-row tiles: bf16, K-major A, MN-major B, 64 columns");
+#pragma unroll
+    for (int k = 0; k < KSTEPS; k++)
+      wgmma_bf16_n256<1, 0>(&acc[0][0], db + (uint64_t)(k * B_STEP), da + (uint64_t)(k * A_STEP), (first && k == 0) ? 0u : 1u);
+  } else {
+#pragma unroll
+    for (int k = 0; k < KSTEPS; k++) {
+      const uint32_t sc = (first && k == 0) ? 0u : 1u;
+#pragma unroll
+      for (int h = 0; h < BM / 64; h++) {
+        const uint64_t a = da + (uint64_t)(h * (8192 >> 4) + k * A_STEP), b = db + (uint64_t)(k * B_STEP);
+        if constexpr (TF32) {
+          if constexpr (BN == 128) wgmma_tf32_n128(acc[h], a, b, sc);
+          else wgmma_tf32_n64(acc[h], a, b, sc);
+        } else {
+          if constexpr (BN == 128) wgmma_bf16_n128<A_MN ? 1 : 0, B_MN ? 1 : 0>(acc[h], a, b, sc);
+          else wgmma_bf16_n64<A_MN ? 1 : 0, B_MN ? 1 : 0>(acc[h], a, b, sc);
+        }
+      }
+    }
+  }
+}
+
+template <int BN, int BM>
+__device__ __forceinline__ void acc_to_smem(const float (&acc)[BM / 64][BN / 2], int hf, float* buf, int ld, int t) {
+  const int w = t >> 5, l = t & 31;
+  if constexpr (BM == 256) {
+    const float* a = &acc[0][0];
+    float* r0 = buf + (2 * (l & 3)) * ld + 16 * w + (l >> 2);
+#pragma unroll
+    for (int j = 0; j < 16; j++) {
+      const int jj = 16 * hf + j;
+#pragma unroll
+      for (int e = 0; e < 2; e++) {
+        r0[(8 * j + e) * ld] = a[4 * jj + e];
+        r0[(8 * j + e) * ld + 8] = a[4 * jj + 2 + e];
+      }
+    }
+  } else {
 #pragma unroll
     for (int h = 0; h < 2; h++) {
-      const uint64_t a = da + (uint64_t)(h * (8192 >> 4) + k * A_STEP), b = db + (uint64_t)(k * B_STEP);
-      if constexpr (TF32) {
-        if constexpr (BN == 128) wgmma_tf32_n128(acc[h], a, b, sc);
-        else wgmma_tf32_n64(acc[h], a, b, sc);
-      } else {
-        if constexpr (BN == 128) wgmma_bf16_n128<A_MN ? 1 : 0, B_MN ? 1 : 0>(acc[h], a, b, sc);
-        else wgmma_bf16_n64<A_MN ? 1 : 0, B_MN ? 1 : 0>(acc[h], a, b, sc);
+      float* r0 = buf + (64 * h + 16 * w + (l >> 2)) * ld + 2 * (l & 3);
+      const float* a = acc[2 * hf + h];
+#pragma unroll
+      for (int j = 0; j < BN / 8; j++) {
+        *reinterpret_cast<float2*>(r0 + 8 * j) = make_float2(a[4 * j], a[4 * j + 1]);
+        *reinterpret_cast<float2*>(r0 + 8 * ld + 8 * j) = make_float2(a[4 * j + 2], a[4 * j + 3]);
       }
-    }
-  }
-}
-
-template <int BN>
-__device__ __forceinline__ void acc_to_smem(const float (&acc)[2][BN / 2], float* buf, int ld, int t) {
-  const int w = t >> 5, l = t & 31;
-#pragma unroll
-  for (int h = 0; h < 2; h++) {
-    float* r0 = buf + (64 * h + 16 * w + (l >> 2)) * ld + 2 * (l & 3);
-#pragma unroll
-    for (int j = 0; j < BN / 8; j++) {
-      *reinterpret_cast<float2*>(r0 + 8 * j) = make_float2(acc[h][4 * j], acc[h][4 * j + 1]);
-      *reinterpret_cast<float2*>(r0 + 8 * ld + 8 * j) = make_float2(acc[h][4 * j + 2], acc[h][4 * j + 3]);
     }
   }
 }
@@ -168,10 +199,12 @@
 constexpr int A_STAGE_BYTES = BLOCK_M * ROW_BYTES;
 constexpr int NUM_THREADS = 384;
 
-template <int BN> struct Cfg {
+template <int BN, int BM = BLOCK_M> struct Cfg {
+  static_assert(BM == 128 || (BM == 256 && BN == 64), "tile shapes: 128 x 64, 128 x 128, 256 x 64");
+  static constexpr int A_STAGE_BYTES = BM * ROW_BYTES;
   static constexpr int B_STAGE_BYTES = BN * ROW_BYTES;
   static constexpr int STAGE_BYTES = A_STAGE_BYTES + B_STAGE_BYTES;
-  static constexpr int STAGES = (BN == 128) ? 4 : 7;
+  static constexpr int STAGES = (BM == 256 || BN == 128) ? 4 : 7;
   static constexpr int ACC_LD = BN + 4;
   static constexpr int ACC_BYTES = BLOCK_M * ACC_LD * 4;
   static constexpr int SMEM_BYTES = STAGES * STAGE_BYTES + ACC_BYTES + 1024  + 512 ;
@@ -187,9 +220,9 @@
   uint64_t* bres_bar;
 };
 
-template <int BN>
+template <int BN, int BM = BLOCK_M>
 __device__ __forceinline__ Smem smem_setup(uint8_t* smem_raw) {
-  using C_ = Cfg<BN>;
+  using C_ = Cfg<BN, BM>;
   Smem s;
   s.ring = reinterpret_cast<uint8_t*>((reinterpret_cast<uintptr_t>(smem_raw) + 1023) & ~(uintptr_t)1023);
   s.accs = reinterpret_cast<float*>(s.ring + C_::STAGES * C_::STAGE_BYTES);
@@ -212,19 +245,20 @@
   return s;
 }
 
-template <bool TF32, int BN, bool A_MN, bool B_MN>
+template <bool TF32, int BN, bool A_MN, bool B_MN, int BM = BLOCK_M>
 __device__ __forceinline__ void mma_loop(const Smem& sm, int num_tiles, int tiles_mn, int splits, int kb_per_split, int nkb_total,
                                          bool bres) {
-  using C_ = Cfg<BN>;
+  using C_ = Cfg<BN, BM>;
+  static_assert(BM == 128 || !A_MN, "256-row tiles take a K-major A");
   const int wt = threadIdx.x - 128;
   const uint32_t smem0 = smem_u32(sm.ring);
   const uint64_t da0 = A_MN ? make_desc(smem0, 64 * 128, 1024) : make_desc(smem0, 0, 1024);
-  const uint64_t db0 = B_MN ? make_desc(smem0 + A_STAGE_BYTES, 64 * 128, 1024) : make_desc(smem0 + A_STAGE_BYTES, 0, 1024);
-  uint32_t it = 0, lt = 0;
+  const uint64_t db0 = B_MN ? make_desc(smem0 + C_::A_STAGE_BYTES, 64 * 128, 1024) : make_desc(smem0 + C_::A_STAGE_BYTES, 0, 1024);
+  uint32_t it = 0, lh = 0;
   if (bres) mbar_wait(sm.bres_bar, 0);
   const uint64_t da0r = make_desc(smem0 + BRES_B_BYTES, 0, 1024), db0r = make_desc(smem0, 0, 1024);
-  float acc[2][BN / 2];
-  for (int t = blockIdx.x; t < num_tiles; t += gridDim.x, lt++) {
+  float acc[BM / 64][BN / 2];
+  for (int t = blockIdx.x; t < num_tiles; t += gridDim.x) {
     const int z = (splits == 1) ? 0 : t / tiles_mn;
     const int kb0 = z * kb_per_split, kb1 = min(kb0 + kb_per_split, nkb_total);
     int prev = -1;
@@ -235,24 +269,27 @@
       const uint64_t stage_off = (uint64_t)((uint32_t)s * (uint32_t)(C_::STAGE_BYTES >> 4));
       const uint64_t a_off = bres ? (uint64_t)((uint32_t)s * (uint32_t)(A_STAGE_BYTES >> 4)) : stage_off;
       const uint64_t b_off = bres ? (uint64_t)((uint32_t)kb * (uint32_t)((64 * 128) >> 4)) : stage_off;
-      fence_regs(acc[0]);
-      fence_regs(acc[1]);
+#pragma unroll
+      for (int h = 0; h < BM / 64; h++) fence_regs(acc[h]);
       wgmma_fence();
-      wgmma_kblock<TF32, BN, A_MN, B_MN>(acc, (bres ? da0r : da0) + a_off, (bres ? db0r : db0) + b_off, kb == kb0);
+      wgmma_kblock<TF32, BN, A_MN, B_MN, BM>(acc, (bres ? da0r : da0) + a_off, (bres ? db0r : db0) + b_off, kb == kb0);
       wgmma_commit();
       wgmma_wait<1>();
-      fence_regs(acc[0]);
-      fence_regs(acc[1]);
+#pragma unroll
+      for (int h = 0; h < BM / 64; h++) fence_regs(acc[h]);
       if (prev >= 0) mbar_arrive(&sm.empty_bar[prev]);
       prev = s;
     }
     wgmma_wait<0>();
-    fence_regs(acc[0]);
-    fence_regs(acc[1]);
+#pragma unroll
+    for (int h = 0; h < BM / 64; h++) fence_regs(acc[h]);
     if (prev >= 0) mbar_arrive(&sm.empty_bar[prev]);
-    mbar_wait(sm.acc_empty_bar, (lt & 1) ^ 1);
-    acc_to_smem<BN>(acc, sm.accs, C_::ACC_LD, wt);
-    mbar_arrive(sm.acc_full_bar);
+#pragma unroll
+    for (int hf = 0; hf < BM / 128; hf++, lh++) {
+      mbar_wait(sm.acc_empty_bar, (lh & 1) ^ 1);
+      acc_to_smem<BN, BM>(acc, hf, sm.accs, C_::ACC_LD, wt);
+      mbar_arrive(sm.acc_full_bar);
+    }
   }
 }
 
@@ -363,11 +400,12 @@
   return P2PVG_OK;
 }
 
-template <auto KERN, int BN, typename... Args>
+template <auto KERN, int BN, int BM = BLOCK_M, typename... Args>
 int launch_persistent(long long tiles, cudaStream_t st, const char* what, Args... args) {
+  constexpr int SMEM_BYTES = Cfg<BN, BM>::SMEM_BYTES;
   static bool smem_attr_set = false;
   if (!smem_attr_set) {
-    const cudaError_t e = cudaFuncSetAttribute(KERN, cudaFuncAttributeMaxDynamicSharedMemorySize, Cfg<BN>::SMEM_BYTES);
+    const cudaError_t e = cudaFuncSetAttribute(KERN, cudaFuncAttributeMaxDynamicSharedMemorySize, SMEM_BYTES);
     if (e != cudaSuccess) {
       p2pvg_set_error("%s: cudaFuncSetAttribute: %s", what, cudaGetErrorString(e));
       return P2PVG_ERR_CUDA;
@@ -375,7 +413,7 @@
     smem_attr_set = true;
   }
   const int sms = driver().sms;
-  KERN<<<(int)(tiles < sms ? tiles : sms), NUM_THREADS, Cfg<BN>::SMEM_BYTES, st>>>(args...);
+  KERN<<<(int)(tiles < sms ? tiles : sms), NUM_THREADS, SMEM_BYTES, st>>>(args...);
   return p2pvg_check_launch(what);
 }
 
```

After: 218,700, median of 6. +3.4%, better.
